# marcin-ochman/modular-slam

Measured on AMD Instinct MI355X. Metric: ORB keypoints extracted+matched /sec, 640×480 RGB-D, 1/2/4/8 GPU; HBM GB/s vs roofline, higher is better.
Workload: dtype u8

## Files before the change

modular-slam_amd/csrc/api.hip:

```cpp
#include "context.hpp"

#include <cfloat>
#include <climits>
#include <cmath>
#include <cstdio>
#include <cstring>
#include <cstdlib>
#include <algorithm>

using namespace mslam;

static thread_local std::string g_create_error;

#define ENTER(c)                                                                                                       \
    do                                                                                                                 \
    {                                                                                                                  \
        if(!(c))                                                                                                       \
            return MSLAM_HIP_E_INVALID;                                                                                \
        MSLAM_CHK(c, hipSetDevice((c)->p.device));                                                                     \
    } while(0)

static inline int cv_round_f(float v) { return (int)lrintf(v); }
static inline int cv_floor_f(float v)
{
    int i = (int)v;
    return i - (i > v);
}
static inline uint32_t sat_coef(float v)
{
    int iv = cv_round_f(v);
    iv = iv < SHRT_MIN ? SHRT_MIN : iv > SHRT_MAX ? SHRT_MAX : iv;
    return (uint32_t)(iv & 0xFFFF);
}

static void resize_table(int ssize, int dsize, bool clamp, std::vector<int32_t>& ofs, std::vector<uint32_t>& coef)
{
    const double inv_scale = (double)dsize / ssize;
    const double scale = 1. / inv_scale;
    for(int d = 0; d < dsize; ++d)
    {
        float f = (float)((d + 0.5) * scale - 0.5);
        int s = cv_floor_f(f);
        f -= s;
        if(clamp)
        {
            if(s < 0)
                f = 0, s = 0;
            if(s >= ssize - 1)
                f = 0, s = ssize - 1;
        }
        ofs.push_back(s);
        coef.push_back(sat_coef((1.f - f) * 2048) | (sat_coef(f * 2048) << 16));
    }
}

static void gaussian_taps_fixed(int taps[7])
{
    const int n = 7, n2 = 3;
    const double sigma = 2.0, scale2x = -0.125 / (sigma * sigma);
    double values[3], sum = 0;
    for(int i = 0, x = 1 - n; i < n2; ++i, x += 2)
    {
        values[i] = std::exp((double)(x * x) * scale2x);
        sum += values[i];
    }
    sum = sum * 2 + 1;
    const double mul1 = 1.0 / sum;
    double err = 0;
    long total = 0;
    for(int i = 0; i < n2; ++i)
    {
        const double adj = values[i] * mul1 * 256.0 + err;
        const long v0 = lrint(adj);
        err = adj - (double)v0;
        taps[i] = taps[n - 1 - i] = (int)v0;
        total += 2 * v0;
    }
    taps[n2] = (int)(256 - total);
}

static bool umax_table(int* out16)
{
    static const int expect[16] = {15, 15, 15, 15, 14, 14, 14, 13, 13, 12, 11, 10, 9, 8, 6, 3};
    int u[17] = {0};
    const int hp = 15;
    const unsigned vmax = (unsigned)std::floor(hp * std::sqrt(2.0) / 2 + 1);
    const unsigned vmin = (unsigned)std::ceil(hp * std::sqrt(2.0) / 2);
    for(unsigned v = 0; v <= vmax; ++v)
        u[v] = (int)std::round(std::sqrt((double)(hp * hp) - (double)(v * v)));
    for(unsigned v = hp, v0 = 0; vmin <= v; --v)
    {
        while(u[v0] == u[v0 + 1])
            ++v0;
        u[v] = (int)v0;
        ++v0;
    }
    std::memcpy(out16, u, sizeof(expect));
    return std::memcmp(u, expect, sizeof(expect)) == 0;
}

static void build_orient_weights(const int* umax, uint32_t* w )
{
    std::memset(w, 0, 2 * 256 * sizeof(uint32_t));
    for(int t = 0; t < 31 * 8; ++t)
    {
        const int v = t / 8 - 15, c = t % 8;
        for(int j = 0; j < 4; ++j)
        {
            const int u = -15 + 4 * c + j;
            const int au = u < 0 ? -u : u, av = v < 0 ? -v : v;
            if(au <= 15 && au <= umax[av])
            {
                w[t] |= (uint32_t)(uint8_t)(int8_t)u << (8 * j);
                w[256 + t] |= (uint32_t)(uint8_t)(int8_t)v << (8 * j);
            }
        }
    }
}

static int build_geometry(mslam_hip_ctx* c)
{
    const mslam_hip_params& p = c->p;
    Geometry& g = c->geom;
    g.n_levels = p.n_levels;
    g.W = p.width;
    g.H = p.height;
    g.blur_tiled = 0;
    float scale[kMaxLevels];
    scale[0] = 1.0f;
    for(int l = 1; l < p.n_levels; ++l)
        scale[l] = p.scale_factor * scale[l - 1];
    unsigned offset = 0;
    c->cells.clear();
    for(int l = 0; l < p.n_levels; ++l)
    {
        LevelGeom& lv = g.lv[l];
        const double s = scale[l];
        lv.w = l == 0 ? p.width : (int)std::round(p.width * 1.0 / s);
        lv.h = l == 0 ? p.height : (int)std::round(p.height * 1.0 / s);
        lv.scale = scale[l];
        if(lv.w <= 2 * kBorder + kOverlap || lv.h <= 2 * kBorder + kOverlap)
            return fail(c, MSLAM_HIP_E_INVALID,
                        "pyramid level " + std::to_string(l) + " is smaller than the 19-px border + one cell");
        if(lv.w > 4095 + kBorder || lv.h > 4095 + kBorder)
            return fail(c, MSLAM_HIP_E_INVALID, "frames larger than 4096 px per side are not supported");
        lv.pitch = (lv.w + kTileW - 1) & ~(kTileW - 1);
        lv.offset = (int)offset;
        offset += ((unsigned)lv.pitch * ((lv.h + kTileH - 1) & ~(kTileH - 1)) + 255u) & ~255u;
        lv.bw = lv.w - 2 * kBorder;
        lv.bh = lv.h - 2 * kBorder;

        const unsigned min_b = kBorder, max_bx = lv.w - kBorder, max_by = lv.h - kBorder;
        const unsigned num_cols = (max_bx - min_b) / kCell + 1, num_rows = (max_by - min_b) / kCell + 1;
        lv.cell_base = (int)c->cells.size();
        for(unsigned i = 0; i < num_rows; ++i)
        {
            const unsigned min_y = min_b + i * kCell;
            if(max_by - kOverlap <= min_y)
                continue;
            unsigned max_y = min_y + kCell + kOverlap;
            if(max_by < max_y)
                max_y = max_by;
            for(unsigned j = 0; j < num_cols; ++j)
            {
                const unsigned min_x = min_b + j * kCell;
                if(max_bx - kOverlap <= min_x)
                    continue;
                unsigned max_x = min_x + kCell + kOverlap;
                if(max_bx < max_x)
                    max_x = max_bx;
                CellDesc cd{};
                cd.level = (int16_t)l;
                cd.cw = (int16_t)(max_x - min_x);
                cd.ch = (int16_t)(max_y - min_y);
                cd.x0 = (int16_t)min_x;
                cd.y0 = (int16_t)min_y;
                cd.ox = (int16_t)(j * kCell);
                cd.oy = (int16_t)(i * kCell);
                c->cells.push_back(cd);
            }
        }
        lv.n_cells = (int)c->cells.size() - lv.cell_base;
        if(lv.n_cells > 2048)
            return fail(c, MSLAM_HIP_E_INVALID, "more than 2048 FAST cells on one level");

        lv.bsx = (lv.w + 3) / 4;

        const int min_x = kBorder, max_x = lv.w - kBorder, min_y = kBorder, max_y = lv.h - kBorder;
        const double ratio = (double)(max_x - min_x) / (max_y - min_y);
        if(ratio > 1)
        {
            lv.nxg = (int)std::round(ratio);
            lv.nyg = 1;
            lv.delta_x = (double)(max_x - min_x) / lv.nxg;
            lv.delta_y = max_y - min_y;
        }
        else
        {
            lv.nxg = 1;
            lv.nyg = (int)std::round(1 / ratio);
            lv.delta_x = max_x - min_y;
            lv.delta_y = (double)(max_y - min_y) / lv.nyg;
        }
        if(lv.nxg * lv.nyg > 64)
            return fail(c, MSLAM_HIP_E_INVALID, "aspect ratio beyond 64:1 is not supported");
    }
    g.slab = offset + 256;
    g.n_cells = (int)c->cells.size();
    return MSLAM_HIP_OK;
}

static int build_geometry_cv(mslam_hip_ctx* c)
{
    const mslam_hip_params& p = c->p;
    Geometry& g = c->geom;
    g.n_levels = p.n_levels;
    g.W = p.width;
    g.H = p.height;
    g.blur_tiled = 0;
    const double sf = (double)p.scale_factor;
    unsigned offset = 0;
    c->cells.clear();
    for(int l = 0; l < p.n_levels; ++l)
    {
        LevelGeom& lv = g.lv[l];
        lv = LevelGeom{};
        lv.scale = (float)std::pow(sf, (double)l);
        const float inv = 1.0f / lv.scale;
        lv.w = cv_round_f((float)p.width * inv);
        lv.h = cv_round_f((float)p.height * inv);
        if(lv.w < 16 || lv.h < 16)
            return fail(c, MSLAM_HIP_E_INVALID, "pyramid level " + std::to_string(l) + " is smaller than 16 px");
        if(lv.w > 4095 || lv.h > 4095)
            return fail(c, MSLAM_HIP_E_INVALID, "frames larger than 4095 px per side are not supported");
        lv.pitch = (lv.w + kTileW - 1) & ~(kTileW - 1);
        lv.offset = (int)offset;
        offset += ((unsigned)lv.pitch * ((lv.h + kTileH - 1) & ~(kTileH - 1)) + 255u) & ~255u;
        lv.bw = lv.w - 2 * kBorder;
        lv.bh = lv.h - 2 * kBorder;
        lv.bsx = (lv.w + 3) / 4;
    }
    g.slab = offset + 256;
    g.n_cells = 0;
    const float factor = (float)(1.0 / sf);
    float desired = (float)p.n_features * (1 - factor) / (1 - (float)std::pow((double)factor, (double)p.n_levels));
    int sum = 0;
    for(int l = 0; l < p.n_levels - 1; ++l)
    {
        c->cv_quota[l] = cv_round_f(desired);
        sum += c->cv_quota[l];
        desired *= factor;
    }
    c->cv_quota[p.n_levels - 1] = std::max(p.n_features - sum, 0);
    return MSLAM_HIP_OK;
}

static void exact_axis(int ssize, int dsize, std::vector<int32_t>& ofs, std::vector<uint32_t>& coef, int& dmin, int& dmax)
{
    const double scale = 1.0 / ((double)dsize / (double)ssize);
    dmin = 0;
    dmax = dsize;
    for(int d = 0; d < dsize; ++d)
    {
        const double fval = scale * ((double)d + 0.5) - 0.5;
        const int ival = (int)std::floor(fval);
        int o = 0;
        uint32_t c0 = 256, c1 = 0;
        if(ival >= 0 && ssize > 1)
        {
            if(ival < ssize - 1)
            {
                o = ival;
                c1 = (uint32_t)lrint((fval - (double)ival) * 256.0);
                c0 = 256 - c1;
            }
            else
            {
                o = ssize - 2;
                c0 = 0, c1 = 256;
                dmax = std::min(dmax, d);
            }
        }
        else
            dmin = std::max(dmin, d + 1);
        ofs.push_back(o);
        coef.push_back(c0 | (c1 << 16));
    }
}

extern "C" {

void mslam_hip_default_params(mslam_hip_params* p)
{
    std::memset(p, 0, sizeof(*p));
    p->width = 640;
    p->height = 480;
    p->max_batch = 1;
    p->n_levels = 8;
    p->scale_factor = 1.2f;
    p->ini_fast_thr = 20;
    p->min_fast_thr = 7;
    p->min_node_area = 1000;
    p->max_keypoints = 8192;
    p->max_candidates = 16384;
    p->device = 0;
    p->stream = nullptr;
    p->detector = MSLAM_HIP_DETECTOR_DISTRIBUTED;
    p->n_features = 1000;
    p->edge_threshold = 31;
}

int mslam_hip_abi_version(void) { return MSLAM_HIP_ABI_VERSION; }

const char* mslam_hip_last_error(const mslam_hip_ctx* ctx) { return ctx ? ctx->err.c_str() : g_create_error.c_str(); }

void mslam_hip_destroy(mslam_hip_ctx* c)
{
    if(!c)
        return;
    if(c->stream)
        (void)hipStreamSynchronize(c->stream);
    if(c->match_graph)
        (void)hipGraphExecDestroy(c->match_graph);
    for(auto& e : c->detect_graph)
        if(e)
            (void)hipGraphExecDestroy(e);
    if(c->stream_m)
        (void)hipStreamSynchronize(c->stream_m);
    for(auto& o : c->out)
    {
        if(o.ev_detect)
            (void)hipEventDestroy(o.ev_detect);
        if(o.ev_match)
            (void)hipEventDestroy(o.ev_match);
    }
    if(c->stream_m)
        (void)hipStreamDestroy(c->stream_m);
    for(auto& t : c->timers)
    {
        (void)hipEventDestroy(t.start);
        (void)hipEventDestroy(t.stop);
    }
    for(int k = 0; k < 4; ++k)
    {
        if(c->blur_stream[k])
        {
            (void)hipStreamSynchronize(c->blur_stream[k]);
            (void)hipStreamDestroy(c->blur_stream[k]);
        }
        if(c->ev_blur_fork[k])
            (void)hipEventDestroy(c->ev_blur_fork[k]);
        if(c->ev_blur_join[k])
            (void)hipEventDestroy(c->ev_blur_join[k]);
    }
    if(c->ev_fork)
        (void)hipEventDestroy(c->ev_fork);
    for(int k = 0; k < 4; ++k)
    {
        if(c->ev_join[k])
            (void)hipEventDestroy(c->ev_join[k]);
        if(c->side[k])
        {
            (void)hipStreamSynchronize(c->side[k]);
            (void)hipStreamDestroy(c->side[k]);
        }
    }
    if(c->bow)
        bow_destroy(c->bow);
    if(c->reloc)
        reloc_destroy(c->reloc);
    if(c->own_stream && c->stream)
        (void)hipStreamDestroy(c->stream);
    delete c;
}

static void build_quad_table(const std::vector<int32_t>& ofs, const std::vector<uint32_t>& coef, size_t x0, int dw,
                             int max_batch, std::vector<uint4>& qt, size_t& start_out, int& need_out)
{
    const int nq = (dw + 3) / 4;
    const size_t start = qt.size() / 3;
    bool ok = true;
    int need = 0;
    for(int q = 0; q < nq && ok; ++q)
    {
        const int first = ofs[x0 + 4 * q];
        const uint32_t base = (uint32_t)first & ~3u;
        uint32_t sel[4], cf[4], flags = 0;
        for(int k = 0; k < 4; ++k)
        {
            const int dx = std::min(4 * q + k, dw - 1);
            const int shift = ofs[x0 + dx] - (int)base;
            const uint32_t a0 = coef[x0 + dx] & 0xFFFF, a1 = coef[x0 + dx] >> 16;
            if(shift < 0 || shift > 10 || a0 > 0xFFF || a1 > 0xFFF)
                ok = false;
            const int upper = shift > 6 ? 1 : 0;
            flags |= (uint32_t)upper << k;
            sel[k] = 0x0c010c00u + (uint32_t)(shift - 4 * upper) * 0x00010001u;
            cf[k] = a0 | (a1 << 16);
        }
        need |= (int)flags;
        qt.push_back(make_uint4(base, flags, sel[0], sel[1]));
        qt.push_back(make_uint4(sel[2], sel[3], cf[0], cf[1]));
        qt.push_back(make_uint4(cf[2], cf[3], 0, 0));
    }
    if(!ok || (size_t)max_batch * nq >= (1u << 22))
    {
        qt.resize(start * 3);
        start_out = SIZE_MAX;
        return;
    }
    start_out = start;
    need_out = need;
}

static int create_impl(mslam_hip_ctx* c)
{
    const mslam_hip_params& p = c->p;
    const bool has_detector = !(p.width == 0 && p.height == 0);
    if((has_detector && (p.width <= 0 || p.height <= 0)) || p.max_batch < 1 || p.n_levels < 1 || p.n_levels > kMaxLevels ||
       !(p.scale_factor > 1.0f) || p.ini_fast_thr < 0 || p.ini_fast_thr > 255 || p.min_fast_thr < 0 ||
       p.min_fast_thr > p.ini_fast_thr || p.max_keypoints < 1 || p.max_keypoints > 65535 || p.max_candidates < 1 ||
       p.max_candidates > (1 << 22))
        return fail(c, MSLAM_HIP_E_INVALID, "invalid parameters");
    const bool cv_mode = p.detector == MSLAM_HIP_DETECTOR_CV_ORB;
    if((p.detector != MSLAM_HIP_DETECTOR_DISTRIBUTED && !cv_mode) ||
       (cv_mode && (p.n_features < 0 || p.edge_threshold < 19 || p.edge_threshold > 1024)))
        return fail(c, MSLAM_HIP_E_INVALID, "invalid detector parameters (cv::ORB mode needs edge_threshold >= 19: "
                                            "the descriptor pattern reaches 19 px)");
    int umax[16];
    if(!umax_table(umax))
        return fail(c, MSLAM_HIP_E_INVALID, "u_max table self-check failed");
    int taps[7];
    gaussian_taps_fixed(taps);
    static const int expect_taps[7] = {18, 34, 48, 56, 48, 34, 18};
    if(std::memcmp(taps, expect_taps, sizeof(taps)) != 0)
        return fail(c, MSLAM_HIP_E_INVALID, "gaussian tap self-check failed");
    set_blur_taps(taps);

    int rc = !has_detector ? MSLAM_HIP_OK : cv_mode ? build_geometry_cv(c) : build_geometry(c);
    if(rc)
        return rc;
    const Geometry& g = c->geom;

    int n_dev = 0;
    if(hipGetDeviceCount(&n_dev) != hipSuccess || n_dev <= 0)
        return fail(c, MSLAM_HIP_E_RUNTIME, "no HIP device available (the product path has no CPU fallback)");
    MSLAM_CHK(c, hipSetDevice(p.device));
    if(p.stream)
        c->stream = (hipStream_t)p.stream;
    else
    {
        MSLAM_CHK(c, hipStreamCreateWithFlags(&c->stream, hipStreamNonBlocking));
        c->own_stream = true;
    }

    {
        if(const char* ge = getenv("MSLAM_HIP_GRAPH"))
            c->use_graph = atoi(ge) != 0;
        const char* e = getenv("MSLAM_HIP_STREAMS");
        c->n_side = e ? std::max(1, std::min(atoi(e), 4)) : 2;
        MSLAM_CHK(c, hipEventCreateWithFlags(&c->ev_fork, hipEventDisableTiming));
        for(int k = 0; k < c->n_side; ++k)
        {
            MSLAM_CHK(c, hipStreamCreateWithFlags(&c->side[k], hipStreamNonBlocking));
            MSLAM_CHK(c, hipEventCreateWithFlags(&c->ev_join[k], hipEventDisableTiming));
        }
        const char* fb = getenv("MSLAM_HIP_FORK_BLUR");
        c->fork_blur = fb && atoi(fb) != 0;
        for(int k = 0; k < 4 && c->fork_blur; ++k)
        {
            MSLAM_CHK(c, hipStreamCreateWithFlags(&c->blur_stream[k], hipStreamNonBlocking));
            MSLAM_CHK(c, hipEventCreateWithFlags(&c->ev_blur_fork[k], hipEventDisableTiming));
            MSLAM_CHK(c, hipEventCreateWithFlags(&c->ev_blur_join[k], hipEventDisableTiming));
        }
    }
    if(has_detector && cv_mode)
    {
        std::vector<int32_t> ofs;
        std::vector<uint32_t> coef;
        c->cv_x.assign(p.n_levels, 0);
        c->cv_y.assign(p.n_levels, 0);
        c->cv_range.assign(p.n_levels, std::array<int, 4>{0, 0, 0, 0});
        c->cv_window12.assign(p.n_levels, 0);
        for(int l = 1; l < p.n_levels; ++l)
        {
            c->cv_x[l] = ofs.size();
            exact_axis(g.lv[l - 1].w, g.lv[l].w, ofs, coef, c->cv_range[l][0], c->cv_range[l][1]);
            c->cv_y[l] = ofs.size();
            exact_axis(g.lv[l - 1].h, g.lv[l].h, ofs, coef, c->cv_range[l][2], c->cv_range[l][3]);
            bool ok = true;
            const int dw = g.lv[l].w;
            for(int q = 0; q * 4 < dw && ok; ++q)
            {
                const int base = ofs[c->cv_x[l] + 4 * q] & ~3;
                for(int k = 0; k < 4; ++k)
                {
                    const int o = ofs[c->cv_x[l] + std::min(4 * q + k, dw - 1)];
                    ok = ok && o >= base && o + 1 - base <= 11;
                }
                ok = ok && base + 12 <= g.lv[l - 1].pitch;
            }
            c->cv_window12[l] = ok ? 1 : 0;
        }
        {
            std::vector<uint4> qt;
            c->rs_q.assign(p.n_levels, SIZE_MAX);
            c->rs_need.assign(p.n_levels, 0);
            for(int l = 1; l < p.n_levels; ++l)
                build_quad_table(ofs, coef, c->cv_x[l], g.lv[l].w, p.max_batch, qt, c->rs_q[l], c->rs_need[l]);
            qt.push_back(make_uint4(0, 0, 0, 0));
            MSLAM_CHK(c, c->d_rs_qt.alloc(qt.size()));
            MSLAM_CHK(c, hipMemcpy(c->d_rs_qt, qt.data(), qt.size() * 16, hipMemcpyHostToDevice));
        }
        ofs.push_back(0);
        coef.push_back(0);
        MSLAM_CHK(c, c->d_cv_ofs.alloc(ofs.size()));
        MSLAM_CHK(c, c->d_cv_coef.alloc(coef.size()));
        MSLAM_CHK(c, hipMemcpy(c->d_cv_ofs, ofs.data(), ofs.size() * 4, hipMemcpyHostToDevice));
        MSLAM_CHK(c, hipMemcpy(c->d_cv_coef, coef.data(), coef.size() * 4, hipMemcpyHostToDevice));
    }
    if(has_detector && !cv_mode)
    {
    MSLAM_CHK(c, c->d_cells.alloc(c->cells.size()));
    MSLAM_CHK(c, hipMemcpy(c->d_cells, c->cells.data(), c->cells.size() * sizeof(CellDesc), hipMemcpyHostToDevice));
    {
        std::vector<int32_t> ofs;
        std::vector<uint32_t> coef;
        c->rs_x.assign(p.n_levels, 0);
        c->rs_y.assign(p.n_levels, 0);
        for(int l = 1; l < p.n_levels; ++l)
        {
            c->rs_x[l] = ofs.size();
            resize_table(g.lv[l - 1].w, g.lv[l].w, true, ofs, coef);
            c->rs_y[l] = ofs.size();
            resize_table(g.lv[l - 1].h, g.lv[l].h, false, ofs, coef);
        }
        std::vector<uint4> qt;
        c->rs_q.assign(p.n_levels, SIZE_MAX);
        c->rs_need.assign(p.n_levels, 0);
        for(int l = 1; l < p.n_levels; ++l)
            build_quad_table(ofs, coef, c->rs_x[l], g.lv[l].w, p.max_batch, qt, c->rs_q[l], c->rs_need[l]);
        qt.push_back(make_uint4(0, 0, 0, 0));
        MSLAM_CHK(c, c->d_rs_qt.alloc(qt.size()));
        MSLAM_CHK(c, hipMemcpy(c->d_rs_qt, qt.data(), qt.size() * 16, hipMemcpyHostToDevice));
        ofs.push_back(0);
        coef.push_back(0);
        MSLAM_CHK(c, c->d_rs_ofs.alloc(ofs.size()));
        MSLAM_CHK(c, c->d_rs_coef.alloc(coef.size()));
        MSLAM_CHK(c, hipMemcpy(c->d_rs_ofs, ofs.data(), ofs.size() * 4, hipMemcpyHostToDevice));
        MSLAM_CHK(c, hipMemcpy(c->d_rs_coef, coef.data(), coef.size() * 4, hipMemcpyHostToDevice));
    }
    }
    MSLAM_CHK(c, c->d_ratio_thr.alloc(257));
    {
        uint32_t w[2 * 256];
        build_orient_weights(umax, w);
        MSLAM_CHK(c, c->d_orient_w.alloc(2 * 256));
        MSLAM_CHK(c, hipMemcpy(c->d_orient_w, w, sizeof(w), hipMemcpyHostToDevice));
    }

    const size_t B = (size_t)p.max_batch, L = (size_t)p.n_levels, cap = (size_t)p.max_candidates;
    const size_t K = (size_t)p.max_keypoints;
    MSLAM_CHK(c, c->h_out.alloc(16 + K * 52));
    MSLAM_CHK(c, c->d_flags.alloc(1));
    MSLAM_CHK(c, hipMemset(c->d_flags, 0, 4));
    if(has_detector)
    {
    {
        uint32_t ok = 0;
        launch_denorm_selfcheck(c->d_flags, c->stream);
        MSLAM_CHK(c, hipGetLastError());
        MSLAM_CHK(c, hipMemcpyAsync(&ok, c->d_flags, 4, hipMemcpyDeviceToHost, c->stream));
        MSLAM_CHK(c, hipStreamSynchronize(c->stream));
        MSLAM_CHK(c, hipMemset(c->d_flags, 0, 4));
        if(ok != 1u)
            return fail(c, MSLAM_HIP_E_RUNTIME, "v_pk_minimum3_f16 / v_pk_maximum3_f16 do not preserve f16 denormals in this build "
                                                "(the FAST score kernels need .amdhsa_float_denorm_mode_16_64 3): refusing to run");
    }
    MSLAM_CHK(c, c->d_stage.alloc((size_t)p.width * p.height * 3));
    MSLAM_CHK(c, c->d_pyr.alloc(B * g.slab + 256));
    MSLAM_CHK(c, c->d_blur.alloc(B * g.slab + 256));
    {
        {
            const char* e = getenv("MSLAM_HIP_FUSED_LEVELS");
            const int want = e ? atoi(e) : kMaxLevels;
            const char* k = getenv("MSLAM_HIP_LEVEL_K6");
            const char* ks = getenv("MSLAM_HIP_LEVEL_K6_SMALL");
            c->level_k6_small = ks ? std::max(0, atoi(ks)) : 0;
            {
                const char* lc = getenv("MSLAM_HIP_LEVEL_CHAIN");
                const char* lf = getenv("MSLAM_HIP_LEVEL_CHAIN_FRAMES");
                const char* lw = getenv("MSLAM_HIP_LEVEL_CHAIN_WAVES");
                const char* lk = getenv("MSLAM_HIP_LEVEL_CHAIN_K6");
                c->level_chain = lc ? atoi(lc) : 0;
                c->level_chain_frames = lf ? std::max(1, std::min(64, atoi(lf))) : 2;
                c->level_chain_waves = lw ? atoi(lw) : 8;
                if(c->level_chain_waves != 4)
                    c->level_chain_waves = 8;
                c->level_chain_k6 = lk ? std::max(1, std::min(9, atoi(lk))) : 9;
            }
            c->level_k6 = k ? std::max(1, atoi(k)) : 9;
            const bool fits = (p.width & 3) == 0 && (double)B * p.width * p.height * 3 < 4294967296.0 &&
                              (double)B * g.slab < 4294901760.0  && (size_t)B * (p.width / 4) < (1u << 22) && p.height >= 8;
            int n_fused = fits ? 1 : 0;
            while(n_fused >= 1 && n_fused < p.n_levels && c->rs_q[n_fused] != SIZE_MAX && g.lv[n_fused].h >= 8 &&
                  (size_t)B * ((g.lv[n_fused].w + 3) / 4) < (1u << 22))
                ++n_fused;
            c->fused_levels = std::max(0, std::min(want, n_fused));
            const char* t = getenv("MSLAM_HIP_TILED_BLUR");
            c->geom.blur_tiled = c->fused_levels == p.n_levels && !(t && atoi(t) == 0) ? 1 : 0;
        }
        std::vector<BlurWave> bw;
        build_blur_waves(g, c->fused_levels, bw);
        c->blur_wpf = (int)bw.size();
        if(!bw.empty())
        {
            MSLAM_CHK(c, c->d_blur_waves.alloc(bw.size()));
            MSLAM_CHK(c, hipMemcpy(c->d_blur_waves, bw.data(), bw.size() * sizeof(BlurWave), hipMemcpyHostToDevice));
        }
    }
    MSLAM_CHK(c, c->d_cell_cnt.alloc(B * g.n_cells));
    MSLAM_CHK(c, c->d_cell_kp.alloc(B * g.n_cells * (size_t)kCellCap));
    QuadArgs& q = c->quad;
    MSLAM_CHK(c, c->q_cand.alloc(B * L * cap));
    MSLAM_CHK(c, c->q_cand_cnt.alloc(B * L));
    MSLAM_CHK(c, c->q_sel.alloc(B * L * cap));
    MSLAM_CHK(c, c->q_sel_cnt.alloc(B * L));
    MSLAM_CHK(c, c->q_kp_node.alloc(B * L * cap));
    MSLAM_CHK(c, c->q_nodes_a.alloc(B * L * cap));
    MSLAM_CHK(c, c->q_nodes_b.alloc(B * L * cap));
    MSLAM_CHK(c, c->q_ncnt_a.alloc(B * L * cap));
    MSLAM_CHK(c, c->q_ncnt_b.alloc(B * L * cap));
    MSLAM_CHK(c, c->q_child_cnt.alloc(B * L * cap * 4));
    MSLAM_CHK(c, c->q_ninfo.alloc(B * L * cap));
    MSLAM_CHK(c, c->q_best.alloc(B * L * cap));
    q.cand = c->q_cand, q.cand_cnt = c->q_cand_cnt, q.sel = c->q_sel, q.sel_cnt = c->q_sel_cnt, q.kp_node = c->q_kp_node;
    q.nodes_a = c->q_nodes_a, q.nodes_b = c->q_nodes_b, q.ncnt_a = c->q_ncnt_a, q.ncnt_b = c->q_ncnt_b;
    q.child_cnt = c->q_child_cnt, q.ninfo = c->q_ninfo, q.best = c->q_best;
    q.cell_cnt = c->d_cell_cnt;
    q.cell_kp = c->d_cell_kp;
    q.flags = c->d_flags;
    q.cand_cap = p.max_candidates;
    q.min_size = p.min_node_area;
    }

    for(auto& o : c->out)
    {
        MSLAM_CHK(c, o.xy.alloc((B + 1) * K * 2));
        MSLAM_CHK(c, o.desc.alloc((B + 1) * K * 32));
        MSLAM_CHK(c, o.octave.alloc((B + 1) * K));
        MSLAM_CHK(c, o.angle.alloc((B + 1) * K));
        MSLAM_CHK(c, o.response.alloc((B + 1) * K));
        MSLAM_CHK(c, o.count.alloc(B + 1));
        MSLAM_CHK(c, hipMemset(o.count, 0, (B + 1) * 4));
        MSLAM_CHK(c, o.idx0.alloc(B * K));
        MSLAM_CHK(c, o.idx1.alloc(B * K));
        MSLAM_CHK(c, o.dist0.alloc(B * K));
        MSLAM_CHK(c, o.dist1.alloc(B * K));
        MSLAM_CHK(c, o.mfrom.alloc(B * K));
        MSLAM_CHK(c, o.mto.alloc(B * K));
        MSLAM_CHK(c, o.mcount.alloc(B));
        MSLAM_CHK(c, hipMemset(o.mcount, 0, B * 4));
        MSLAM_CHK(c, hipEventCreateWithFlags(&o.ev_detect, hipEventDisableTiming));
        MSLAM_CHK(c, hipEventCreateWithFlags(&o.ev_match, hipEventDisableTiming));
    }
    MSLAM_CHK(c, hipStreamCreateWithFlags(&c->stream_m, hipStreamNonBlocking));
    {
        const char* e = getenv("MSLAM_HIP_OVERLAP_MATCH");
        c->overlap_match = !(e && atoi(e) == 0);
        auto on = [](const char* name) { const char* v = getenv(name); return !v || atoi(v) != 0; };
        c->knob_mirror_results = on("MSLAM_HIP_MIRROR_RESULTS");
        c->knob_zero_copy = on("MSLAM_HIP_ZERO_COPY_FRAME");
        c->knob_match_graph = on("MSLAM_HIP_MATCH_GRAPH");
        const char* zm = getenv("MSLAM_HIP_ZERO_COPY_MAX_BYTES");
        c->zero_copy_max_bytes = zm ? (size_t)atoll(zm) : (size_t)1200000;
        const char* m = getenv("MSLAM_HIP_MATCHER");
        c->matcher_kind = (m && std::strcmp(m, "popcount") == 0) ? MSLAM_HIP_MATCHER_POPCOUNT : MSLAM_HIP_MATCHER_AUTO;
    }
    c->cur = 0;
    MSLAM_CHK(c, hipDeviceSynchronize());
    return MSLAM_HIP_OK;
}

int mslam_hip_create(const mslam_hip_params* p, mslam_hip_ctx** out)
{
    if(!p || !out)
    {
        g_create_error = "null argument";
        return MSLAM_HIP_E_INVALID;
    }
    *out = nullptr;
    mslam_hip_ctx* c = new mslam_hip_ctx();
    c->p = *p;
    const int rc = create_impl(c);
    if(rc != MSLAM_HIP_OK)
    {
        g_create_error = c->err;
        mslam_hip_destroy(c);
        return rc;
    }
    *out = c;
    return MSLAM_HIP_OK;
}

constexpr int kMinChunk = 8;

static int check_flags(mslam_hip_ctx* c)
{
    uint32_t f = 0;
    MSLAM_CHK(c, hipStreamSynchronize(c->stream_m));
    MSLAM_CHK(c, hipMemcpyAsync(&f, c->d_flags, 4, hipMemcpyDeviceToHost, c->stream));
    MSLAM_CHK(c, hipStreamSynchronize(c->stream));
    if(f == 0)
        return MSLAM_HIP_OK;
    MSLAM_CHK(c, hipMemsetAsync(c->d_flags, 0, 4, c->stream));
    std::string m = "capacity exceeded:";
    if(f & kFlagCandOverflow)
        m += " FAST candidates on a level > max_candidates;";
    if(f & kFlagKpOverflow)
        m += " keypoints in a frame > max_keypoints;";
    if(f & kFlagQuadNoConverge)
        m += " quadtree pass limit;";
    if(f & kFlagDbFull)
        m += " the BoW database is full (mslam_hip_bow_db_reserve);";
    if(f & kFlagBowPackOverflow)
        m += " a BoW vector has more words than the exchange format's k_max;";
    if(f & kFlagPackOverflow)
        m += " packed batch results larger than the buffer given to mslam_hip_pack_batch_dev (header.bytes);";
    if(f & kFlagUnionOverflow)
        m += " a union of store entries has more distinct landmarks than max_keypoints (mslam_hip_kf_union_dev);";
    return fail(c, MSLAM_HIP_E_CAPACITY, m);
}

int mslam_hip_sync(mslam_hip_ctx* c)
{
    ENTER(c);
    return check_flags(c);
}

__global__ __launch_bounds__(256) void k_pack_results(const float* __restrict__ xy, const uint8_t* __restrict__ desc,
                                                      const int32_t* __restrict__ octave, const float* __restrict__ angle,
                                                      const float* __restrict__ response, const int32_t* __restrict__ count,
                                                      const uint32_t* __restrict__ flags, uint8_t* __restrict__ h, int K)
{
    const int n = min(max(*count, 0), K);
    const int tid = blockIdx.x * 256 + threadIdx.x, nt = gridDim.x * 256;
    if(tid == 0)
    {
        reinterpret_cast<int32_t*>(h)[0] = *count;
        reinterpret_cast<uint32_t*>(h)[1] = *flags;
    }
    uint2* h_xy = reinterpret_cast<uint2*>(h + 16);
    uint2* h_desc = reinterpret_cast<uint2*>(h + 16 + (size_t)K * 8);
    uint32_t* h_oct = reinterpret_cast<uint32_t*>(h + 16 + (size_t)K * 40);
    uint32_t* h_ang = h_oct + K;
    uint32_t* h_resp = h_ang + K;
    for(int i = tid; i < 4 * n; i += nt)
        h_desc[i] = reinterpret_cast<const uint2*>(desc)[i];
    for(int i = tid; i < n; i += nt)
    {
        h_xy[i] = reinterpret_cast<const uint2*>(xy)[i];
        h_oct[i] = reinterpret_cast<const uint32_t*>(octave)[i];
        h_ang[i] = reinterpret_cast<const uint32_t*>(angle)[i];
        h_resp[i] = reinterpret_cast<const uint32_t*>(response)[i];
    }
}

__global__ __launch_bounds__(256) void k_carry_prev(uint4* __restrict__ dst, const uint4* __restrict__ src, int32_t* __restrict__ dst_count,
                                                    const int32_t* __restrict__ src_count, int K)
{
    const int n = min(max(*src_count, 0), K);
    const int tid = blockIdx.x * 256 + threadIdx.x;
    if(tid == 0)
        *dst_count = *src_count;
    for(int i = tid; i < 2 * n; i += gridDim.x * 256)
        dst[i] = src[i];
}

static void enqueue_resize_blur(mslam_hip_ctx* c, int l, const int32_t* yofs, const uint32_t* ycoef, int exact, int f0, int nf,
                                int k6, hipStream_t cs, ResizeBlurArgs* chain_out = nullptr)
{
    const Geometry& g = c->geom;
    const LevelGeom &sl = g.lv[l - 1], &dl = g.lv[l];
    ResizeBlurArgs ra{};
    ra.pyr = c->d_pyr;
    ra.blur = c->d_blur;
    ra.slab = g.slab;
    ra.src_off = sl.offset, ra.sh = sl.h, ra.spitch = sl.pitch;
    ra.dst_off = dl.offset, ra.dw = dl.w, ra.dh = dl.h, ra.dpitch = dl.pitch;
    ra.qt = c->d_rs_qt + 3 * c->rs_q[l];
    ra.yofs = yofs;
    ra.ycoef = ycoef;
    ra.frame0 = f0, ra.n_frames = nf;
    ra.quads = (dl.w + 3) / 4;
    ra.inv_quads = 1.0f / (float)ra.quads;
    if(k6 == 0 && dl.h >= 380)
        k6 = 1;
    ra.k6 = std::max(k6 == 0 ? 0 : 1, std::min(std::min(k6, 9), (dl.h - 2) / 6));
    {
        const long waves_x = ((long)nf * ra.quads + 61) / 62;
        while(ra.k6 > 2 && waves_x * ((dl.h + 6 * ra.k6 + 1) / (6 * ra.k6 + 2)) < 2048)
            --ra.k6;
    }
    ra.need_mask = c->rs_need[l];
    ra.exact = exact;
    ra.blur_tiled = g.blur_tiled;
    ra.always_load = nf < 8 ? 1 : 0;
    ra.bk = make_blur_k();
    if(chain_out)
    {
        *chain_out = ra;
        return;
    }
    launch_resize_blur(ra, cs);
}

static int enqueue_detect(mslam_hip_ctx* c, const uint8_t* d_bgr, int n_frames)
{
    const Geometry& g = c->geom;
    const size_t K = (size_t)c->p.max_keypoints;
    hipStream_t s = c->stream;
    const int k6_batch = n_frames >= 8 ? c->level_k6 : c->level_k6_small;
    const int n_chunks = (c->profiling || n_frames < 2 * kMinChunk) ? 1 : std::min<int>(c->n_side, n_frames / kMinChunk);
    if(n_chunks > 1)
        MSLAM_CHK(c, hipEventRecord(c->ev_fork, s));
    for(int k = 0; k < n_chunks; ++k)
    {
        const int f0 = (int)((long long)n_frames * k / n_chunks), f1 = (int)((long long)n_frames * (k + 1) / n_chunks);
        const int nf = f1 - f0;
        hipStream_t cs = n_chunks > 1 ? c->side[k] : s;
        if(n_chunks > 1)
            MSLAM_CHK(c, hipStreamWaitEvent(cs, c->ev_fork, 0));
        const bool cv_mode = c->p.detector == MSLAM_HIP_DETECTOR_CV_ORB;
        bool chained = false;
        if(c->level_chain && !cv_mode && nf >= 8 && c->fused_levels == g.n_levels && g.n_levels <= kChainLevels && g.blur_tiled)
        {
            StageScope t(c, "levels", cs);
            GrayBlurArgs ga{};
            ga.bgr = d_bgr;
            ga.pyr = c->d_pyr;
            ga.blur = c->d_blur;
            ga.W = g.W, ga.H = g.H, ga.pitch = g.lv[0].pitch;
            ga.slab = g.slab;
            ga.n_frames = nf, ga.frame0 = f0;
            ga.quads = g.W / 4;
            ga.inv_quads = 1.0f / (float)ga.quads;
            ga.k6 = 1;
            ga.blur_tiled = g.blur_tiled;
            ga.bk = make_blur_k();
            ResizeBlurArgs lv[kChainLevels - 1];
            for(int l = 1; l < g.n_levels; ++l)
                enqueue_resize_blur(c, l, c->d_rs_ofs + c->rs_y[l], c->d_rs_coef + c->rs_y[l], 0, f0, nf, k6_batch, cs, &lv[l - 1]);
            chained = launch_level_chain(ga, lv, g.n_levels - 1, c->level_chain_frames, c->level_chain_waves, c->level_chain_k6, cs);
        }
        if(!chained)
        {
            StageScope t(c, "gray", cs);
            if(c->fused_levels >= 1)
            {
                GrayBlurArgs ga{};
                ga.bgr = d_bgr;
                ga.pyr = c->d_pyr;
                ga.blur = c->d_blur;
                ga.W = g.W, ga.H = g.H, ga.pitch = g.lv[0].pitch;
                ga.slab = g.slab;
                ga.n_frames = nf, ga.frame0 = f0;
                ga.quads = g.W / 4;
                ga.inv_quads = 1.0f / (float)ga.quads;
                ga.k6 = std::max(k6_batch == 0 && g.H < 380 ? 0 : 1, std::min(k6_batch, (g.H - 2) / 6));
                ga.blur_tiled = g.blur_tiled;
                ga.bk = make_blur_k();
                launch_gray_blur(ga, cs);
            }
            else
                launch_gray(d_bgr, c->d_pyr, g, f0, nf, cs);
        }
        if(cv_mode)
        {
            {
                StageScope t(c, "resize", cs);
                for(int l = 1; l < g.n_levels; ++l)
                {
                    const LevelGeom &sl = g.lv[l - 1], &dl = g.lv[l];
                    if(l < c->fused_levels)
                    {
                        enqueue_resize_blur(c, l, c->d_cv_ofs + c->cv_y[l], c->d_cv_coef + c->cv_y[l], 1, f0, nf, k6_batch, cs);
                        continue;
                    }
                    if(c->rs_q[l] != SIZE_MAX)
                    {
                        ResizeColArgs ca{};
                        ca.pyr = c->d_pyr;
                        ca.slab = g.slab;
                        ca.src_off = sl.offset, ca.sh = sl.h, ca.spitch = sl.pitch;
                        ca.dst_off = dl.offset, ca.dw = dl.w, ca.dh = dl.h, ca.dpitch = dl.pitch;
                        ca.qt = c->d_rs_qt + 3 * c->rs_q[l];
                        ca.yofs = c->d_cv_ofs + c->cv_y[l];
                        ca.ycoef = c->d_cv_coef + c->cv_y[l];
                        ca.frame0 = f0, ca.n_frames = nf;
                        ca.quads = (dl.w + 3) / 4;
                        ca.inv_quads = 1.0f / (float)ca.quads;
                        ca.R = 8;
                        ca.need_mask = c->rs_need[l];
                        ca.exact = 1;
                        launch_resize_col(ca, cs);
                        continue;
                    }
                    ExactResizeArgs ra{};
                    ra.pyr = c->d_pyr;
                    ra.slab = g.slab;
                    ra.src_off = sl.offset, ra.sw = sl.w, ra.sh = sl.h, ra.spitch = sl.pitch;
                    ra.dst_off = dl.offset, ra.dw = dl.w, ra.dh = dl.h, ra.dpitch = dl.pitch;
                    ra.xofs = c->d_cv_ofs + c->cv_x[l];
                    ra.xcoef = c->d_cv_coef + c->cv_x[l];
                    ra.yofs = c->d_cv_ofs + c->cv_y[l];
                    ra.ycoef = c->d_cv_coef + c->cv_y[l];
                    ra.xmin = c->cv_range[l][0], ra.xmax = c->cv_range[l][1];
                    ra.ymin = c->cv_range[l][2], ra.ymax = c->cv_range[l][3];
                    ra.window12 = c->cv_window12[l];
                    ra.frame0 = f0;
                    launch_resize_exact(ra, nf, cs);
                }
            }
            CvSelectArgs sa{};
            sa.cand = c->quad.cand, sa.cand_cnt = c->quad.cand_cnt;
            sa.tmp_kp = c->quad.kp_node, sa.tmp_resp = reinterpret_cast<float*>(c->quad.ninfo);
            sa.sel = c->quad.sel, sa.sel_resp = reinterpret_cast<float*>(c->quad.best), sa.sel_cnt = c->quad.sel_cnt;
            sa.flags = c->d_flags;
            sa.cand_cap = c->p.max_candidates;
            sa.edge = c->p.edge_threshold;
            sa.std_order = c->cv_order == MSLAM_HIP_CV_ORDER_LIBSTDCXX ? 1 : 0;
            for(int l = 0; l < g.n_levels; ++l)
                sa.quota[l] = c->cv_quota[l];
            {
                StageScope t(c, "fast", cs);
                launch_zero_u32(c->quad.cand_cnt + (size_t)f0 * g.n_levels, nf * g.n_levels, cs);
                launch_fast_tiles(c->d_pyr, g, c->p.ini_fast_thr, sa, f0, nf, cs);
            }
            {
                StageScope t(c, "select", cs);
                launch_cv_select(c->d_pyr, g, sa, f0, nf, cs);
            }
        }
        else
        {
        if(!chained)
        {
            StageScope t(c, "resize", cs);
            for(int l = 1; l < g.n_levels; ++l)
            {
                if(l < c->fused_levels)
                {
                    enqueue_resize_blur(c, l, c->d_rs_ofs + c->rs_y[l], c->d_rs_coef + c->rs_y[l], 0, f0, nf, k6_batch, cs);
                    continue;
                }
                if(c->rs_q[l] != SIZE_MAX)
                {
                    const LevelGeom &sl = g.lv[l - 1], &dl = g.lv[l];
                    ResizeColArgs ra{};
                    ra.pyr = c->d_pyr;
                    ra.slab = g.slab;
                    ra.src_off = sl.offset;
                    ra.sh = sl.h;
                    ra.spitch = sl.pitch;
                    ra.dst_off = dl.offset;
                    ra.dw = dl.w;
                    ra.dh = dl.h;
                    ra.dpitch = dl.pitch;
                    ra.qt = c->d_rs_qt + 3 * c->rs_q[l];
                    ra.yofs = c->d_rs_ofs + c->rs_y[l];
                    ra.ycoef = c->d_rs_coef + c->rs_y[l];
                    ra.frame0 = f0;
                    ra.n_frames = nf;
                    ra.quads = (dl.w + 3) / 4;
                    ra.inv_quads = 1.0f / (float)ra.quads;
                    ra.R = 8;
                    ra.need_mask = c->rs_need[l];
                    launch_resize_col(ra, cs);
                }
                else
                    launch_resize(c->d_pyr, g, l, c->d_rs_ofs + c->rs_x[l], c->d_rs_coef + c->rs_x[l],
                                  c->d_rs_ofs + c->rs_y[l], c->d_rs_coef + c->rs_y[l], f0, nf, cs);
            }
        }
        {
            StageScope t(c, "fast", cs);
            launch_fast(c->d_pyr, g, c->d_cells, c->d_cell_cnt, c->d_cell_kp, c->p.ini_fast_thr, c->p.min_fast_thr, f0,
                        nf, cs);
        }
        const bool blur_needed = c->fused_levels < g.n_levels;
        const bool forked = c->fork_blur && !c->profiling && blur_needed;
        if(forked)
        {
            MSLAM_CHK(c, hipEventRecord(c->ev_blur_fork[k], cs));
            MSLAM_CHK(c, hipStreamWaitEvent(c->blur_stream[k], c->ev_blur_fork[k], 0));
            {
                StageScope t(c, "blur", c->blur_stream[k]);
                launch_blur(c->d_pyr, c->d_blur, g, c->d_blur_waves, c->blur_wpf, f0, nf, c->blur_stream[k]);
            }
            MSLAM_CHK(c, hipEventRecord(c->ev_blur_join[k], c->blur_stream[k]));
        }
        {
            StageScope t(c, "quadtree", cs);
            launch_quadtree(g, c->quad, f0, nf, cs);
        }
        if(forked)
            MSLAM_CHK(c, hipStreamWaitEvent(cs, c->ev_blur_join[k], 0));
        else if(blur_needed)
        {
            StageScope t(c, "blur", cs);
            launch_blur(c->d_pyr, c->d_blur, g, c->d_blur_waves, c->blur_wpf, f0, nf, cs);
        }
        }
        if(cv_mode && c->fused_levels < g.n_levels)
        {
            StageScope t(c, "blur", cs);
            launch_blur(c->d_pyr, c->d_blur, g, c->d_blur_waves, c->blur_wpf, f0, nf, cs);
        }
        {
            StageScope t(c, "describe", cs);
            DescArgs a{};
            a.pyr = c->d_pyr;
            a.blur = c->d_blur;
            a.sel = c->quad.sel;
            a.sel_cnt = c->quad.sel_cnt;
            a.orient_w = c->d_orient_w;
            a.cand_cap = c->p.max_candidates;
            a.max_kp = c->p.max_keypoints;
            a.xy = cur_out(c).xy + K * 2;
            a.desc = cur_out(c).desc + K * 32;
            a.octave = cur_out(c).octave + K;
            a.angle = cur_out(c).angle + K;
            a.response = cur_out(c).response + K;
            a.count = cur_out(c).count + 1;
            a.flags = c->d_flags;
            if(cv_mode)
            {
                a.sel_resp = reinterpret_cast<const float*>(c->quad.best);
                a.cv_mode = 1;
            }
            if(c->mirror_results && n_frames == 1)
                a.h_mirror = c->h_out.dev();
            launch_describe(g, a, f0, nf, cs);
        }
        if(n_chunks > 1)
        {
            MSLAM_CHK(c, hipEventRecord(c->ev_join[k], cs));
            MSLAM_CHK(c, hipStreamWaitEvent(s, c->ev_join[k], 0));
        }
    }
    MSLAM_CHK(c, hipGetLastError());
    return MSLAM_HIP_OK;
}

static int detect_prologue(mslam_hip_ctx* c)
{
    const size_t K = (size_t)c->p.max_keypoints;
    hipStream_t s = c->stream;
    if(!c->inplace_timing)
        c->timers_used = 0;
    if(c->n_last > 0)
    {
        const int prev = c->cur, nxt = prev ^ 1;
        if(c->out[nxt].match_pending)
        {
            MSLAM_CHK(c, hipStreamWaitEvent(s, c->out[nxt].ev_match, 0));
            c->out[nxt].match_pending = false;
        }
        const size_t last = (size_t)c->n_last;
        hipLaunchKernelGGL(k_carry_prev, dim3(16), dim3(256), 0, s, reinterpret_cast<uint4*>(c->out[nxt].desc.get()),
                           reinterpret_cast<const uint4*>(c->out[prev].desc + last * K * 32), c->out[nxt].count,
                           c->out[prev].count + last, (int)K);
        MSLAM_CHK(c, hipGetLastError());
        c->have_prev = true;
        c->cur = nxt;
    }
    return MSLAM_HIP_OK;
}

int mslam_hip_detect_batch_dev(mslam_hip_ctx* c, const uint8_t* d_bgr, int n_frames)
{
    ENTER(c);
    if(c->p.width == 0)
        return fail(c, MSLAM_HIP_E_INVALID, "detect_batch_dev: this context was created without a detector (0 x 0)");
    if(!d_bgr || n_frames < 1 || n_frames > c->p.max_batch)
        return fail(c, MSLAM_HIP_E_INVALID, "detect_batch_dev: n_frames outside [1, max_batch]");
    int rc = detect_prologue(c);
    if(rc)
        return rc;
    rc = enqueue_detect(c, d_bgr, n_frames);
    if(rc)
        return rc;
    MSLAM_CHK(c, hipEventRecord(c->out[c->cur].ev_detect, c->stream));
    c->n_last = n_frames;
    ++c->detect_seq;
    return MSLAM_HIP_OK;
}

int mslam_hip_get_batch_view(mslam_hip_ctx* c, mslam_hip_batch_view* v)
{
    if(!c || !v)
        return MSLAM_HIP_E_INVALID;
    const size_t K = (size_t)c->p.max_keypoints;
    v->n_frames = c->n_last;
    v->capacity = c->p.max_keypoints;
    v->xy = cur_out(c).xy + K * 2;
    v->desc = cur_out(c).desc + K * 32;
    v->octave = cur_out(c).octave + K;
    v->angle = cur_out(c).angle + K;
    v->response = cur_out(c).response + K;
    v->count = cur_out(c).count + 1;
    v->match_from = cur_out(c).mfrom;
    v->match_to = cur_out(c).mto;
    v->match_count = cur_out(c).mcount;
    return MSLAM_HIP_OK;
}

int mslam_hip_detect(mslam_hip_ctx* c, const uint8_t* bgr, int width, int height, int max_out, float* xy,
                     uint8_t* desc, int32_t* octave, float* angle, float* response, int* n_out)
{
    ENTER(c);
    if(n_out)
        *n_out = 0;
    if(!bgr || !n_out || max_out < 0 || (max_out > 0 && (!xy || !desc)))
        return fail(c, MSLAM_HIP_E_INVALID, "detect: null argument");
    if(c->p.width == 0)
        return fail(c, MSLAM_HIP_E_INVALID, "detect: this context was created without a detector (0 x 0)");
    if(width != c->p.width || height != c->p.height)
        return fail(c, MSLAM_HIP_E_INVALID, "detect: frame size differs from the context's");
    const size_t K = (size_t)c->p.max_keypoints;
    uint8_t* h = c->h_out;
    uint8_t* h_xy = h + 16;
    uint8_t* h_desc = h_xy + K * 8;
    uint8_t* h_oct = h_desc + K * 32;
    uint8_t* h_ang = h_oct + K * 4;
    uint8_t* h_resp = h_ang + K * 4;
    const bool mirror_env = c->knob_mirror_results;
    struct MirrorScope
    {
        mslam_hip_ctx* c;
        MirrorScope(mslam_hip_ctx* cc, bool on) : c(cc) { c->mirror_results = on; }
        ~MirrorScope() { c->mirror_results = false; }
    } mirror_scope(c, mirror_env);
    auto enqueue_results = [&]() -> int {
        if(c->mirror_results)
            return MSLAM_HIP_OK;
        const mslam_out_set& o = cur_out(c);
        hipLaunchKernelGGL(k_pack_results, dim3(32), dim3(256), 0, c->stream, o.xy + K * 2, o.desc + K * 32, o.octave + K,
                           o.angle + K, o.response + K, o.count + 1, c->d_flags, c->h_out.dev(), (int)K);
        MSLAM_CHK(c, hipGetLastError());
        return MSLAM_HIP_OK;
    };
    MSLAM_CHK(c, hipStreamSynchronize(c->stream_m));
    int rc = detect_prologue(c);
    if(rc)
        return rc;
    const bool zero_copy = c->knob_zero_copy && (size_t)width * height * 3 <= c->zero_copy_max_bytes;
    const uint8_t* frame_src = c->d_stage;
    if(zero_copy)
    {
        if(!c->h_stage)
        {
            MSLAM_CHK(c, c->h_stage.alloc((size_t)width * height * 3));
        }
        std::memcpy(c->h_stage, bgr, (size_t)width * height * 3);
        frame_src = c->h_stage.dev();
    }
    else
        MSLAM_CHK(c, hipMemcpyAsync(c->d_stage, bgr, (size_t)width * height * 3, hipMemcpyHostToDevice, c->stream));
    if(!c->profiling && !c->inplace_timing && c->use_graph)
    {
        hipGraphExec_t& exec = c->detect_graph[c->cur];
        if(!exec)
        {
            hipGraph_t graph = nullptr;
            MSLAM_CHK(c, hipStreamBeginCapture(c->stream, hipStreamCaptureModeRelaxed));
            rc = enqueue_detect(c, frame_src, 1);
            if(!rc)
                rc = enqueue_results();
            const hipError_t e = hipStreamEndCapture(c->stream, &graph);
            const hipError_t e_inst = (!rc && e == hipSuccess) ? hipGraphInstantiate(&exec, graph, nullptr, nullptr, 0) : hipSuccess;
            if(graph)
                (void)hipGraphDestroy(graph);
            if(e_inst != hipSuccess)
                exec = nullptr;
            if(rc)
                return rc;
            MSLAM_CHK(c, e);
            MSLAM_CHK(c, e_inst);
        }
        MSLAM_CHK(c, hipGraphLaunch(exec, c->stream));
    }
    else
    {
        rc = enqueue_detect(c, frame_src, 1);
        if(rc)
            return rc;
        rc = enqueue_results();
        if(rc)
            return rc;
    }
    MSLAM_CHK(c, hipEventRecord(c->out[c->cur].ev_detect, c->stream));
    c->n_last = 1;
    ++c->detect_seq;
    MSLAM_CHK(c, hipStreamSynchronize(c->stream));
    uint32_t flags;
    int32_t n;
    std::memcpy(&n, h, 4);
    std::memcpy(&flags, h + 4, 4);
    if(flags)
        return check_flags(c);
    *n_out = n;
    if(n > max_out)
        return fail(c, MSLAM_HIP_E_CAPACITY, "detect: max_out smaller than the number of keypoints");
    if(n == 0)
        return MSLAM_HIP_OK;
    std::memcpy(xy, h_xy, (size_t)n * 8);
    std::memcpy(desc, h_desc, (size_t)n * 32);
    if(octave)
        std::memcpy(octave, h_oct, (size_t)n * 4);
    if(angle)
        std::memcpy(angle, h_ang, (size_t)n * 4);
    if(response)
        std::memcpy(response, h_resp, (size_t)n * 4);
    return MSLAM_HIP_OK;
}

static int upload_ratio_table(mslam_hip_ctx* c, double ratio)
{
    if(ratio == c->ratio_cached)
        return MSLAM_HIP_OK;
    int32_t thr[257];
    for(int d1 = 0; d1 <= 256; ++d1)
    {
        int n = 0;
        for(int d0 = 0; d0 <= 256; ++d0)
            if((double)(float)d0 < ratio * (double)(float)d1)
                ++n;
            else
                break;
        thr[d1] = n;
    }
    MSLAM_CHK(c, hipStreamSynchronize(c->stream_m));
    MSLAM_CHK(c, hipMemcpyAsync(c->d_ratio_thr, thr, sizeof(thr), hipMemcpyHostToDevice, c->stream));
    MSLAM_CHK(c, hipStreamSynchronize(c->stream));
    c->ratio_cached = ratio;
    return MSLAM_HIP_OK;
}
__attribute__((visibility("hidden"))) int mslam_ratio_table(mslam_hip_ctx* c, double ratio) { return upload_ratio_table(c, ratio); }

int mslam_hip_match_batch_dev(mslam_hip_ctx* c, double ratio, int chain_previous)
{
    ENTER(c);
    if(c->n_last < 1)
        return fail(c, MSLAM_HIP_E_INVALID, "match_batch_dev: no detect batch to match");
    int rc = upload_ratio_table(c, ratio);
    if(rc)
        return rc;
    const size_t K = (size_t)c->p.max_keypoints;
    const int first = (chain_previous && c->have_prev) ? 0 : 1;
    const int n_pairs = c->n_last - first;
    c->match_seq = c->detect_seq;
    const bool own = c->overlap_match && !c->profiling;
    hipStream_t s = own ? c->stream_m : c->stream;
    if(own)
        MSLAM_CHK(c, hipStreamWaitEvent(s, c->out[c->cur].ev_detect, 0));
    if(first == 1)
        MSLAM_CHK(c, hipMemsetAsync(cur_out(c).mcount, 0, 4, s));
    if(n_pairs > 0)
    {
        MatchArgs m{};
        m.from_desc = cur_out(c).desc + (size_t)(first + 1) * K * 32;
        m.to_desc = cur_out(c).desc + (size_t)first * K * 32;
        m.from_stride = m.to_stride = (long long)K * 32;
        m.from_cnt = cur_out(c).count + first + 1;
        m.to_cnt = cur_out(c).count + first;
        m.cap = c->p.max_keypoints;
        m.cap_from = c->p.max_keypoints;
        m.popcount_only = c->matcher_kind == MSLAM_HIP_MATCHER_POPCOUNT;
        m.idx0 = cur_out(c).idx0 + (size_t)first * K;
        m.idx1 = cur_out(c).idx1 + (size_t)first * K;
        m.dist0 = cur_out(c).dist0 + (size_t)first * K;
        m.dist1 = cur_out(c).dist1 + (size_t)first * K;
        {
            StageScope t(c, "match_knn2", s);
            c->last_match_kernel = launch_match_knn2(m, n_pairs, s);
        }
        RatioArgs r{};
        r.idx0 = m.idx0;
        r.dist0 = m.dist0;
        r.dist1 = m.dist1;
        r.from_cnt = m.from_cnt;
        r.to_cnt = m.to_cnt;
        r.cap = m.cap;
        r.thr = c->d_ratio_thr;
        r.from_idx = cur_out(c).mfrom + (size_t)first * K;
        r.to_idx = cur_out(c).mto + (size_t)first * K;
        r.n_out = cur_out(c).mcount + first;
        {
            StageScope t(c, "ratio_compact", s);
            launch_ratio_compact(r, n_pairs, s);
        }
    }
    MSLAM_CHK(c, hipGetLastError());
    if(own)
    {
        MSLAM_CHK(c, hipEventRecord(c->out[c->cur].ev_match, s));
        c->out[c->cur].match_pending = true;
    }
    return MSLAM_HIP_OK;
}

constexpr int kHostMatchSlices = 8;
static int host_match_prepare(mslam_hip_ctx* c, const uint8_t* from_desc, int n_from, const uint8_t* to_desc, int n_to)
{
    if(n_from > c->hm_from_cap || n_to > c->hm_to_cap)
    {
        MSLAM_CHK(c, hipStreamSynchronize(c->stream));
        const int from_cap = std::max(n_from, std::max(c->hm_from_cap, 2048)), to_cap = std::max(n_to, std::max(c->hm_to_cap, 2048));
        c->hm_from_cap = c->hm_to_cap = 0;
        c->d_hm_to = nullptr;
        if(c->match_graph)
        {
            (void)hipGraphExecDestroy(c->match_graph);
            c->match_graph = nullptr;
        }
        MSLAM_CHK(c, c->d_hm_from.alloc((size_t)(from_cap + to_cap) * 32 + 16));
        MSLAM_CHK(c, c->d_hm_out.alloc((size_t)to_cap * 6 + 4));
        MSLAM_CHK(c, c->d_hm_partial.alloc((size_t)kHostMatchSlices * 2 * to_cap));
        MSLAM_CHK(c, c->h_hm.alloc((size_t)(from_cap + to_cap) * 32 + 16 + ((size_t)to_cap * 2 + 4) * 4));
        c->hm_from_cap = from_cap;
        c->hm_to_cap = to_cap;
    }
    c->d_hm_to = c->d_hm_from + (size_t)n_from * 32;
    if(n_from > 0)
        std::memcpy(c->h_hm, from_desc, (size_t)n_from * 32);
    std::memcpy(c->h_hm + (size_t)n_from * 32, to_desc, (size_t)n_to * 32);
    MSLAM_CHK(c, hipMemcpyAsync(c->d_hm_from, c->h_hm, (size_t)(n_from + n_to) * 32, hipMemcpyHostToDevice, c->stream));
    return MSLAM_HIP_OK;
}

static void host_match_args(mslam_hip_ctx* c, int n_from, int n_to, MatchArgs& m)
{
    const size_t cap = (size_t)c->hm_to_cap;
    m = MatchArgs{};
    m.from_desc = c->d_hm_from;
    m.to_desc = c->d_hm_to;
    m.n_from_fixed = n_from;
    m.n_to_fixed = n_to;
    m.cap = n_to;
    m.idx0 = c->d_hm_out;
    m.idx1 = c->d_hm_out + cap;
    m.dist0 = c->d_hm_out + 2 * cap;
    m.dist1 = c->d_hm_out + 3 * cap;
    m.popcount_only = c->matcher_kind == MSLAM_HIP_MATCHER_POPCOUNT;
    m.partial = c->d_hm_partial;
    m.n_slices = std::max(1, std::min(kHostMatchSlices, (n_from + 255) / 256));
}

static int host_match_graph(mslam_hip_ctx* c, const uint8_t* from_desc, int n_from, const uint8_t* to_desc, int n_to, int* n_out,
                            int32_t* from_idx, int32_t* to_idx)
{
    const size_t fcap = (size_t)c->hm_from_cap, tcap = (size_t)c->hm_to_cap;
    uint8_t* h_cnt = c->h_hm + (fcap + tcap) * 32;
    if(n_from > 0)
        std::memcpy(c->h_hm, from_desc, (size_t)n_from * 32);
    if(n_to > 0)
        std::memcpy(c->h_hm + fcap * 32, to_desc, (size_t)n_to * 32);
    const int32_t counts[4] = {n_from, n_to, 0, 0};
    std::memcpy(h_cnt, counts, sizeof(counts));
    int32_t* res_dev = reinterpret_cast<int32_t*>(c->h_hm.dev() + (fcap + tcap) * 32 + 16);
    const int32_t* res = reinterpret_cast<const int32_t*>(c->h_hm + (fcap + tcap) * 32 + 16);
    if(!c->match_graph || c->match_graph_from_cap != c->hm_from_cap || c->match_graph_to_cap != c->hm_to_cap ||
       c->match_graph_kind != c->matcher_kind)
    {
        if(c->match_graph)
            (void)hipGraphExecDestroy(c->match_graph);
        c->match_graph = nullptr;
        hipGraph_t graph = nullptr;
        MSLAM_CHK(c, hipStreamBeginCapture(c->stream, hipStreamCaptureModeRelaxed));
        hipError_t e = hipMemcpyAsync(c->d_hm_from, c->h_hm, (fcap + tcap) * 32 + 16, hipMemcpyHostToDevice, c->stream);
        const int32_t* d_cnt = reinterpret_cast<const int32_t*>(c->d_hm_from + (fcap + tcap) * 32);
        MatchArgs m{};
        m.from_desc = c->d_hm_from;
        m.to_desc = c->d_hm_from + fcap * 32;
        m.from_cnt = d_cnt;
        m.to_cnt = d_cnt + 1;
        m.cap = (int)tcap;
        m.cap_from = (int)fcap;
        m.idx0 = c->d_hm_out;
        m.idx1 = c->d_hm_out + tcap;
        m.dist0 = c->d_hm_out + 2 * tcap;
        m.dist1 = c->d_hm_out + 3 * tcap;
        m.popcount_only = c->matcher_kind == MSLAM_HIP_MATCHER_POPCOUNT;
        m.partial = c->d_hm_partial;
        m.n_slices = kHostMatchSlices;
        RatioArgs r{};
        r.idx0 = m.idx0;
        r.dist0 = m.dist0;
        r.dist1 = m.dist1;
        r.from_cnt = m.from_cnt;
        r.to_cnt = m.to_cnt;
        r.cap = (int)tcap;
        r.thr = c->d_ratio_thr;
        r.from_idx = res_dev;
        r.to_idx = res_dev + tcap;
        r.n_out = res_dev + 2 * tcap;
        if(launch_match_ratio_single(m, r, c->stream))
            c->last_match_kernel = 1;
        else
        {
            c->last_match_kernel = launch_match_knn2(m, 1, c->stream);
            launch_ratio_compact(r, 1, c->stream);
        }
        const hipError_t e_launch = hipGetLastError();
        const hipError_t e2 = hipStreamEndCapture(c->stream, &graph);
        hipError_t e3 = (e == hipSuccess && e_launch == hipSuccess && e2 == hipSuccess)
                            ? hipGraphInstantiate(&c->match_graph, graph, nullptr, nullptr, 0)
                            : hipSuccess;
        if(graph)
            (void)hipGraphDestroy(graph);
        if(e3 != hipSuccess)
            c->match_graph = nullptr;
        MSLAM_CHK(c, e);
        MSLAM_CHK(c, e_launch);
        MSLAM_CHK(c, e2);
        MSLAM_CHK(c, e3);
        c->match_graph_from_cap = c->hm_from_cap;
        c->match_graph_to_cap = c->hm_to_cap;
        c->match_graph_kind = c->matcher_kind;
        c->match_graph_kernel = c->last_match_kernel;
    }
    c->last_match_kernel = c->match_graph_kernel;
    MSLAM_CHK(c, hipGraphLaunch(c->match_graph, c->stream));
    MSLAM_CHK(c, hipStreamSynchronize(c->stream));
    const int32_t n = res[2 * tcap];
    if(n < 0 || n > n_to || (size_t)n > tcap)
        return fail(c, MSLAM_HIP_E_RUNTIME, "match: the kernel reported an impossible match count");
    std::memcpy(from_idx, res, (size_t)n * 4);
    std::memcpy(to_idx, res + tcap, (size_t)n * 4);
    *n_out = n;
    return MSLAM_HIP_OK;
}

int mslam_hip_join_matcher(mslam_hip_ctx* c)
{
    ENTER(c);
    for(auto& o : c->out)
        if(o.match_pending)
            MSLAM_CHK(c, hipStreamWaitEvent(c->stream, o.ev_match, 0));
    return MSLAM_HIP_OK;
}

int mslam_hip_set_matcher(mslam_hip_ctx* c, int kind)
{
    if(!c)
        return MSLAM_HIP_E_INVALID;
    if(kind != MSLAM_HIP_MATCHER_AUTO && kind != MSLAM_HIP_MATCHER_POPCOUNT)
        return fail(c, MSLAM_HIP_E_INVALID, "set_matcher: unknown kind");
    c->matcher_kind = kind;
    return MSLAM_HIP_OK;
}

int mslam_hip_get_matcher(const mslam_hip_ctx* c) { return c ? c->matcher_kind : -1; }

int mslam_hip_set_cv_keypoint_order(mslam_hip_ctx* c, int order)
{
    ENTER(c);
    if(order != MSLAM_HIP_CV_ORDER_LIBSTDCXX && order != MSLAM_HIP_CV_ORDER_RASTER)
        return fail(c, MSLAM_HIP_E_INVALID, "set_cv_keypoint_order: unknown order");
    if(order == c->cv_order)
        return MSLAM_HIP_OK;
    MSLAM_CHK(c, hipStreamSynchronize(c->stream));
    for(auto& e : c->detect_graph)
        if(e)
        {
            (void)hipGraphExecDestroy(e);
            e = nullptr;
        }
    c->cv_order = order;
    return MSLAM_HIP_OK;
}
int mslam_hip_last_match_kernel(const mslam_hip_ctx* c) { return c ? c->last_match_kernel : -1; }

int mslam_hip_match_knn2(mslam_hip_ctx* c, const uint8_t* from_desc, int n_from, const uint8_t* to_desc, int n_to,
                         int32_t* idx0, int32_t* idx1, int32_t* dist0, int32_t* dist1)
{
    ENTER(c);
    if(n_from < 0 || n_to < 0 || (n_from > 0 && !from_desc) || (n_to > 0 && (!to_desc || !idx0 || !idx1 || !dist0 || !dist1)))
        return fail(c, MSLAM_HIP_E_INVALID, "match_knn2: bad argument");
    if(n_from > 65535)
        return fail(c, MSLAM_HIP_E_INVALID, "match_knn2: more than 65535 train descriptors are not supported");
    if(n_to == 0)
        return MSLAM_HIP_OK;
    int rc = host_match_prepare(c, from_desc, n_from, to_desc, n_to);
    if(rc)
        return rc;
    MatchArgs m;
    host_match_args(c, n_from, n_to, m);
    c->last_match_kernel = launch_match_knn2(m, 1, c->stream);
    MSLAM_CHK(c, hipGetLastError());
    MSLAM_CHK(c, hipMemcpyAsync(idx0, m.idx0, (size_t)n_to * 4, hipMemcpyDeviceToHost, c->stream));
    MSLAM_CHK(c, hipMemcpyAsync(idx1, m.idx1, (size_t)n_to * 4, hipMemcpyDeviceToHost, c->stream));
    MSLAM_CHK(c, hipMemcpyAsync(dist0, m.dist0, (size_t)n_to * 4, hipMemcpyDeviceToHost, c->stream));
    MSLAM_CHK(c, hipMemcpyAsync(dist1, m.dist1, (size_t)n_to * 4, hipMemcpyDeviceToHost, c->stream));
    MSLAM_CHK(c, hipStreamSynchronize(c->stream));
    return MSLAM_HIP_OK;
}

int mslam_hip_match(mslam_hip_ctx* c, const uint8_t* from_desc, int n_from, const uint8_t* to_desc, int n_to,
                    double ratio, int32_t* from_idx, int32_t* to_idx, int* n_out)
{
    ENTER(c);
    if(n_out)
        *n_out = 0;
    if(!n_out || n_from < 0 || n_to < 0 || (n_from > 0 && !from_desc) || (n_to > 0 && (!to_desc || !from_idx || !to_idx)))
        return fail(c, MSLAM_HIP_E_INVALID, "match: bad argument");
    if(n_from > 65535)
        return fail(c, MSLAM_HIP_E_INVALID, "match: more than 65535 train descriptors are not supported");
    if(n_to == 0 || n_from < 2)
        return MSLAM_HIP_OK;
    int rc = upload_ratio_table(c, ratio);
    if(rc)
        return rc;
    const bool graph_env = c->knob_match_graph;
    if(graph_env && c->use_graph && !c->profiling && !c->inplace_timing && c->hm_from_cap >= n_from && c->hm_to_cap >= n_to &&
       c->hm_from_cap + c->hm_to_cap <= 2 * (n_from + n_to) + 2048 && c->hm_from_cap <= 32736)
        return host_match_graph(c, from_desc, n_from, to_desc, n_to, n_out, from_idx, to_idx);
    rc = host_match_prepare(c, from_desc, n_from, to_desc, n_to);
    if(rc)
        return rc;
    if(graph_env && c->use_graph && !c->profiling && !c->inplace_timing && c->hm_from_cap <= 32736 &&
       c->hm_from_cap + c->hm_to_cap <= 2 * (n_from + n_to) + 2048)
    {
        MSLAM_CHK(c, hipStreamSynchronize(c->stream));
        return host_match_graph(c, from_desc, n_from, to_desc, n_to, n_out, from_idx, to_idx);
    }
    MatchArgs m;
    host_match_args(c, n_from, n_to, m);
    c->last_match_kernel = launch_match_knn2(m, 1, c->stream);
    const size_t cap = (size_t)c->hm_to_cap;
    RatioArgs r{};
    r.idx0 = m.idx0;
    r.dist0 = m.dist0;
    r.dist1 = m.dist1;
    r.n_from_fixed = n_from;
    r.n_to_fixed = n_to;
    r.cap = n_to;
    r.thr = c->d_ratio_thr;
    int32_t* res_dev = reinterpret_cast<int32_t*>(c->h_hm.dev() + (size_t)(c->hm_from_cap + c->hm_to_cap) * 32 + 16);
    const int32_t* res = reinterpret_cast<const int32_t*>(c->h_hm + (size_t)(c->hm_from_cap + c->hm_to_cap) * 32 + 16);
    r.from_idx = res_dev;
    r.to_idx = res_dev + cap;
    r.n_out = res_dev + 2 * cap;
    launch_ratio_compact(r, 1, c->stream);
    MSLAM_CHK(c, hipGetLastError());
    MSLAM_CHK(c, hipStreamSynchronize(c->stream));
    const int32_t n = res[2 * cap];
    std::memcpy(from_idx, res, (size_t)n * 4);
    std::memcpy(to_idx, res + cap, (size_t)n * 4);
    *n_out = n;
    return MSLAM_HIP_OK;
}

int mslam_hip_level_geometry(mslam_hip_ctx* c, int* widths, int* heights, float* scales)
{
    if(!c)
        return MSLAM_HIP_E_INVALID;
    for(int l = 0; l < c->geom.n_levels; ++l)
    {
        if(widths)
            widths[l] = c->geom.lv[l].w;
        if(heights)
            heights[l] = c->geom.lv[l].h;
        if(scales)
            scales[l] = c->geom.lv[l].scale;
    }
    return MSLAM_HIP_OK;
}

int mslam_hip_debug_read(mslam_hip_ctx* c, int what, int frame, int level, void* dst, size_t dst_bytes,
                         size_t* n_items)
{
    ENTER(c);
    if(c->p.width == 0 || frame < 0 || frame >= c->p.max_batch || level < 0 || level >= c->geom.n_levels || !dst || !n_items)
        return fail(c, MSLAM_HIP_E_INVALID, "debug_read: bad argument");
    MSLAM_CHK(c, hipStreamSynchronize(c->stream));
    const LevelGeom& lv = c->geom.lv[level];
    if(what == MSLAM_HIP_DBG_PYRAMID || what == MSLAM_HIP_DBG_BLURRED)
    {
        const size_t need = (size_t)lv.w * lv.h;
        *n_items = need;
        if(dst_bytes < need)
            return fail(c, MSLAM_HIP_E_CAPACITY, "debug_read: buffer too small");
        const uint8_t* src = (what == MSLAM_HIP_DBG_PYRAMID ? c->d_pyr : c->d_blur) + (size_t)frame * c->geom.slab + lv.offset;
        if(what == MSLAM_HIP_DBG_BLURRED && c->geom.blur_tiled)
        {
            std::vector<uint8_t> tmp((size_t)lv.pitch * ((lv.h + kTileH - 1) & ~(kTileH - 1)));
            MSLAM_CHK(c, hipMemcpy(tmp.data(), src, tmp.size(), hipMemcpyDeviceToHost));
            uint8_t* out = static_cast<uint8_t*>(dst);
            for(int y = 0; y < lv.h; ++y)
                for(int x = 0; x < lv.w; ++x)
                    out[(size_t)y * lv.w + x] = tmp[tiled_off((unsigned)lv.pitch, x, y)];
            return MSLAM_HIP_OK;
        }
        MSLAM_CHK(c, hipMemcpy2D(dst, lv.w, src, lv.pitch, lv.w, lv.h, hipMemcpyDeviceToHost));
        return MSLAM_HIP_OK;
    }
    if(what == MSLAM_HIP_DBG_CANDIDATES || what == MSLAM_HIP_DBG_SELECTED)
    {
        const size_t slot = (size_t)frame * c->geom.n_levels + level;
        const bool cand = what == MSLAM_HIP_DBG_CANDIDATES;
        uint32_t n = 0;
        MSLAM_CHK(c, hipMemcpy(&n, (cand ? c->quad.cand_cnt : c->quad.sel_cnt) + slot, 4, hipMemcpyDeviceToHost));
        n = std::min<uint32_t>(n, (uint32_t)c->p.max_candidates);
        *n_items = n;
        if(dst_bytes < (size_t)n * 12)
            return fail(c, MSLAM_HIP_E_CAPACITY, "debug_read: buffer too small");
        std::vector<uint32_t> tmp(n);
        if(n)
            MSLAM_CHK(c, hipMemcpy(tmp.data(), (cand ? c->quad.cand : c->quad.sel) + slot * (size_t)c->p.max_candidates,
                                   (size_t)n * 4, hipMemcpyDeviceToHost));
        if(cand && c->p.detector == MSLAM_HIP_DETECTOR_CV_ORB && c->cv_order == MSLAM_HIP_CV_ORDER_LIBSTDCXX && n > (uint32_t)kSelLds)
            std::sort(tmp.begin(), tmp.end());
        float* out = static_cast<float*>(dst);
        for(uint32_t i = 0; i < n; ++i)
        {
            out[3 * i] = (float)kp_x(tmp[i]);
            out[3 * i + 1] = (float)kp_y(tmp[i]);
            out[3 * i + 2] = (float)kp_score(tmp[i]);
        }
        if(c->p.detector == MSLAM_HIP_DETECTOR_CV_ORB && !cand)
        {
            std::vector<float> resp(n);
            if(n)
                MSLAM_CHK(c, hipMemcpy(resp.data(), reinterpret_cast<const float*>(c->quad.best) + slot * (size_t)c->p.max_candidates,
                                       (size_t)n * 4, hipMemcpyDeviceToHost));
            for(uint32_t i = 0; i < n; ++i)
            {
                out[3 * i] += (float)kBorder;
                out[3 * i + 1] += (float)kBorder;
                out[3 * i + 2] = resp[i];
            }
        }
        return MSLAM_HIP_OK;
    }
    if(what == MSLAM_HIP_DBG_CELLS && c->p.detector == MSLAM_HIP_DETECTOR_DISTRIBUTED)
    {
        *n_items = (size_t)lv.n_cells;
        if(dst_bytes < (size_t)lv.n_cells * 24)
            return fail(c, MSLAM_HIP_E_CAPACITY, "debug_read: buffer too small");
        int32_t* out = static_cast<int32_t*>(dst);
        for(int i = 0; i < lv.n_cells; ++i)
        {
            const CellDesc& cd = c->cells[(size_t)lv.cell_base + i];
            const int32_t rec[6] = {cd.x0, cd.y0, cd.cw, cd.ch, cd.ox, cd.oy};
            std::memcpy(out + 6 * i, rec, sizeof(rec));
        }
        return MSLAM_HIP_OK;
    }
    if(what == MSLAM_HIP_DBG_FORMS)
    {
        *n_items = 2;
        if(dst_bytes < 8)
            return fail(c, MSLAM_HIP_E_CAPACITY, "debug_read: buffer too small");
        const int32_t rec[2] = {c->fused_levels, c->geom.blur_tiled};
        std::memcpy(dst, rec, sizeof(rec));
        return MSLAM_HIP_OK;
    }
    return fail(c, MSLAM_HIP_E_INVALID, "debug_read: unknown item");
}

int mslam_hip_debug_counts(mslam_hip_ctx* c, int what, int32_t* out, int n_frames)
{
    ENTER(c);
    if(c->p.width == 0 || !out || n_frames < 1 || (what != MSLAM_HIP_DBG_CANDIDATES && what != MSLAM_HIP_DBG_SELECTED))
        return fail(c, MSLAM_HIP_E_INVALID, "debug_counts: bad argument");
    MSLAM_CHK(c, hipStreamSynchronize(c->stream));
    const int rows = std::min(n_frames, std::max(c->n_last, 1));
    MSLAM_CHK(c, hipMemcpy(out, what == MSLAM_HIP_DBG_CANDIDATES ? c->quad.cand_cnt : c->quad.sel_cnt,
                           (size_t)rows * c->geom.n_levels * 4, hipMemcpyDeviceToHost));
    return MSLAM_HIP_OK;
}

int mslam_hip_copy_to_host(mslam_hip_ctx* c, void* dst_host, const void* src_dev, size_t bytes)
{
    ENTER(c);
    if(!dst_host || !src_dev)
        return fail(c, MSLAM_HIP_E_INVALID, "copy_to_host: null pointer");
    MSLAM_CHK(c, hipStreamSynchronize(c->stream_m));
    MSLAM_CHK(c, hipStreamSynchronize(c->stream));
    MSLAM_CHK(c, hipMemcpy(dst_host, src_dev, bytes, hipMemcpyDeviceToHost));
    return MSLAM_HIP_OK;
}

int mslam_hip_set_profiling(mslam_hip_ctx* c, int enable)
{
    if(!c)
        return MSLAM_HIP_E_INVALID;
    c->profiling = enable == 1;
    c->inplace_timing = enable == 2;
    c->timers_used = 0;
    return MSLAM_HIP_OK;
}

int mslam_hip_get_stage_times(mslam_hip_ctx* c, const char** names, float* ms, int cap, int* n)
{
    ENTER(c);
    if(!n)
        return fail(c, MSLAM_HIP_E_INVALID, "get_stage_times: null output");
    MSLAM_CHK(c, hipStreamSynchronize(c->stream_m));
    MSLAM_CHK(c, hipStreamSynchronize(c->stream));
    int k = 0;
    for(size_t i = 0; i < c->timers_used && k < cap; ++i, ++k)
    {
        float t = 0;
        MSLAM_CHK(c, hipEventElapsedTime(&t, c->timers[i].start, c->timers[i].stop));
        if(names)
            names[k] = c->timers[i].name;
        if(ms)
            ms[k] = t;
    }
    *n = k;
    if(c->inplace_timing)
        c->timers_used = 0;
    return MSLAM_HIP_OK;
}

}
```

modular-slam_amd/csrc/common.hpp:

```cpp
#pragma once
#include <hip/hip_runtime.h>
#include <cstdint>
#include <cstddef>

namespace mslam
{

constexpr int kMaxLevels = 16;
constexpr int kBorder = 19;
constexpr int kCell = 64;
constexpr int kOverlap = 6;
constexpr int kCellCap = 1024;

constexpr size_t al256(size_t x) { return (x + 255) & ~(size_t)255; }

struct LevelGeom
{
    int w, h;
    int pitch;
    int offset;
    float scale;
    int bw, bh;
    int cell_base;
    int n_cells;
    int bsx;
    int nxg, nyg;
    double delta_x, delta_y;
};

struct Geometry
{
    int n_levels;
    int W, H;
    int n_cells;
    int frame0;
    unsigned slab;
    int blur_tiled;
    LevelGeom lv[kMaxLevels];
};

#ifndef MSLAM_TILE_W
#define MSLAM_TILE_W 64
#endif
constexpr int kTileW = MSLAM_TILE_W, kTileH = 128 / kTileW;
constexpr int kTileWLog = kTileW == 64 ? 6 : kTileW == 32 ? 5 : 4, kTileHLog = 7 - kTileWLog;
static_assert(kTileW == 16 || kTileW == 32 || kTileW == 64, "tile width");
__host__ __device__ __forceinline__ unsigned tiled_off(unsigned pitch, int x, int y)
{
    return (unsigned)(y >> kTileHLog) * (pitch * (unsigned)kTileH) + (unsigned)(x >> kTileWLog) * 128u +
           (unsigned)(y & (kTileH - 1)) * (unsigned)kTileW + (unsigned)(x & (kTileW - 1));
}
template <class P>
__device__ __forceinline__ P lds_ptr(uint32_t off)
{
#if defined(__HIP_DEVICE_COMPILE__)
    return (P)off;
#else
    return (P)(uintptr_t)off;
#endif
}
struct CellDesc
{
    int16_t level, cw, ch, pad;
    int16_t x0, y0;
    int16_t ox, oy;
};

constexpr int kBlurRows = 32;

__host__ __device__ inline uint32_t pack_kp(int x, int y, int score) { return ((uint32_t)y << 20) | ((uint32_t)x << 8) | (uint32_t)score; }
__host__ __device__ inline int kp_x(uint32_t p) { return (int)((p >> 8) & 0xFFFu); }
__host__ __device__ inline int kp_y(uint32_t p) { return (int)(p >> 20); }
__host__ __device__ inline int kp_score(uint32_t p) { return (int)(p & 0xFFu); }

enum : uint32_t
{
    kFlagCandOverflow = 1u,
    kFlagKpOverflow = 2u,
    kFlagQuadNoConverge = 4u,
    kFlagBowPackOverflow = 8u,
    kFlagDbFull = 16u,
    kFlagPackOverflow = 32u,
    kFlagUnionOverflow = 64u
};

void launch_gray(const uint8_t* d_bgr, uint8_t* d_pyr, const Geometry& g, int frame0, int n_frames, hipStream_t s);
void launch_resize(uint8_t* d_pyr, const Geometry& g, int level, const int32_t* d_xofs, const uint32_t* d_xcoef,
                   const int32_t* d_yofs, const uint32_t* d_ycoef, int frame0, int n_frames, hipStream_t s);
struct ResizeColArgs
{
    uint8_t* pyr;
    unsigned slab;
    int src_off, sh, spitch, dst_off, dw, dh, dpitch;
    const uint4* qt;
    const int32_t* yofs;
    const uint32_t* ycoef;
    int frame0, n_frames;
    int quads;
    float inv_quads;
    int R;
    int need_mask;
    int exact;
};
void launch_resize_col(const ResizeColArgs& a, hipStream_t s);
void launch_fast(const uint8_t* d_pyr, const Geometry& g, const CellDesc* d_cells, uint32_t* d_cell_cnt,
                 uint32_t* d_cell_kp, int ini_thr, int min_thr, int frame0, int n_frames, hipStream_t s);
void launch_denorm_selfcheck(uint32_t* d_out, hipStream_t s);
struct QuadArgs
{
    const uint32_t* cell_cnt;
    const uint32_t* cell_kp;
    uint32_t* cand;
    uint32_t* cand_cnt;
    uint32_t* sel;
    uint32_t* sel_cnt;
    uint32_t* kp_node;
    uint2* nodes_a;
    uint2* nodes_b;
    uint32_t* ncnt_a;
    uint32_t* ncnt_b;
    uint32_t* child_cnt;
    uint32_t* ninfo;
    uint32_t* best;
    uint32_t* flags;
    int cand_cap;
    unsigned min_size;
};
void launch_quadtree(const Geometry& g, const QuadArgs& a, int frame0, int n_frames, hipStream_t s);
struct BlurK
{
    uint32_t ta[3], tb[4], tc[4];
    uint32_t t01, t23, t45, t6;
};
BlurK make_blur_k();
struct GrayBlurArgs
{
    const uint8_t* bgr;
    uint8_t* pyr;
    uint8_t* blur;
    int W, H, pitch;
    unsigned slab;
    int n_frames, frame0;
    int quads;
    float inv_quads;
    int k6;
    int waves_per_xcd;
    int blur_tiled;
    BlurK bk;
};
void launch_gray_blur(const GrayBlurArgs& a, hipStream_t s);
struct ResizeBlurArgs
{
    uint8_t* pyr;
    uint8_t* blur;
    unsigned slab;
    int src_off, sh, spitch, dst_off, dw, dh, dpitch;
    const uint4* qt;
    const int32_t* yofs;
    const uint32_t* ycoef;
    int frame0, n_frames;
    int quads;
    float inv_quads;
    int k6;
    int need_mask;
    int exact;
    int waves_per_xcd;
    int blur_tiled;
    int always_load;
    BlurK bk;
};
void launch_resize_blur(const ResizeBlurArgs& a, hipStream_t s);
constexpr int kChainLevels = 8;
struct LevelChainArgs
{
    GrayBlurArgs g;
    ResizeBlurArgs lv[kChainLevels - 1];
    int n_lv;
    int G;
    int n_groups, groups_per_xcd;
    int frame0, n_frames;
};
bool launch_level_chain(const GrayBlurArgs& g, const ResizeBlurArgs* lv, int n_lv, int frames_per_group, int waves, int k6_max, hipStream_t s);
struct BlurWave
{
    int level;
    int item0;
    int generic;
    float inv_bsx;
};
void launch_blur(const uint8_t* d_pyr, uint8_t* d_blur, const Geometry& g, const BlurWave* d_waves, int wpf, int frame0, int n_frames,
                 hipStream_t s);
struct DescArgs
{
    const uint8_t* pyr;
    const uint8_t* blur;
    const uint32_t* sel;
    const uint32_t* sel_cnt;
    const uint32_t* orient_w;
    int cand_cap;
    int max_kp;
    float* xy;
    uint8_t* desc;
    int32_t* octave;
    float* angle;
    float* response;
    int32_t* count;
    uint32_t* flags;
    int n_frames = 0;
    const float* sel_resp = nullptr;
    uint8_t* h_mirror = nullptr;
    int cv_mode = 0;
};
void launch_describe(const Geometry& g, const DescArgs& a, int frame0, int n_frames, hipStream_t s);

struct ExactResizeArgs
{
    uint8_t* pyr;
    unsigned slab;
    int src_off, sw, sh, spitch, dst_off, dw, dh, dpitch;
    const int32_t* xofs;
    const uint32_t* xcoef;
    const int32_t* yofs;
    const uint32_t* ycoef;
    int xmin, xmax, ymin, ymax;
    int window12;
    int frame0;
};
void launch_resize_exact(const ExactResizeArgs& a, int n_frames, hipStream_t s);
struct CvSelectArgs
{
    uint32_t* cand;
    uint32_t* cand_cnt;
    uint32_t* tmp_kp;
    float* tmp_resp;
    uint32_t* sel;
    float* sel_resp;
    uint32_t* sel_cnt;
    uint32_t* flags;
    int cand_cap;
    int edge;
    int quota[kMaxLevels];
    int std_order;
};
constexpr int kSelLds = 4096;
constexpr int kSelLdsSmall = 1024;
void launch_zero_u32(uint32_t* p, int n, hipStream_t s);
void launch_fast_tiles(const uint8_t* d_pyr, const Geometry& g, int thr, const CvSelectArgs& a, int frame0, int n_frames,
                       hipStream_t s);
void launch_cv_select(const uint8_t* d_pyr, const Geometry& g, const CvSelectArgs& a, int frame0, int n_frames,
                      hipStream_t s);

struct MatchArgs
{
    const uint8_t* from_desc;
    const uint8_t* to_desc;
    long long from_stride, to_stride;
    const int32_t* from_cnt;
    const int32_t* to_cnt;
    int n_from_fixed, n_to_fixed;
    int cap;
    int32_t* idx0;
    int32_t* idx1;
    int32_t* dist0;
    int32_t* dist1;
    int cap_from = 0;
    int popcount_only = 0;
    uint32_t* partial = nullptr;
    int n_slices = 0;
    int n_pairs = 0, wg_per_pair = 0;
};
int launch_match_knn2(const MatchArgs& a, int n_pairs, hipStream_t s);
struct RatioArgs
{
    const int32_t* idx0;
    const int32_t* dist0;
    const int32_t* dist1;
    const int32_t* from_cnt;
    const int32_t* to_cnt;
    int n_from_fixed, n_to_fixed;
    int cap;
    const int32_t* thr;
    int32_t* from_idx;
    int32_t* to_idx;
    int32_t* n_out;
};
void launch_ratio_compact(const RatioArgs& a, int n_pairs, hipStream_t s);
bool launch_match_ratio_single(const MatchArgs& a, const RatioArgs& r, hipStream_t s);

}
```

modular-slam_amd/csrc/context.hpp:

```cpp
#pragma once
#include "common.hpp"
#include "devmem.hpp"
#include "../../include/mslam_hip.h"
#include <array>
#include <string>
#include <vector>

namespace mslam
{
struct BowState;
void bow_destroy(BowState*);
struct RelocState;
void reloc_destroy(RelocState*);
void set_blur_taps(const int* taps);
void build_blur_waves(const Geometry& g, int first_level, std::vector<BlurWave>& out);

struct StageTimer
{
    const char* name;
    hipEvent_t start, stop;
};
}

struct mslam_out_set
{
    mslam::DevBuf<float> xy;
    mslam::DevBuf<uint8_t> desc;
    mslam::DevBuf<int32_t> octave;
    mslam::DevBuf<float> angle, response;
    mslam::DevBuf<int32_t> count;
    mslam::DevBuf<int32_t> idx0, idx1, dist0, dist1;
    mslam::DevBuf<int32_t> mfrom, mto, mcount;
    hipEvent_t ev_detect = nullptr, ev_match = nullptr;
    bool match_pending = false;
};

struct mslam_hip_ctx
{
    mslam_hip_params p{};
    mslam::Geometry geom{};
    hipStream_t stream = nullptr;
    bool own_stream = false;
    int n_side = 2;
    hipStream_t side[4] = {nullptr, nullptr, nullptr, nullptr};
    hipEvent_t ev_fork = nullptr, ev_join[4] = {nullptr, nullptr, nullptr, nullptr};
    hipStream_t blur_stream[4] = {nullptr, nullptr, nullptr, nullptr};
    hipEvent_t ev_blur_fork[4] = {nullptr, nullptr, nullptr, nullptr}, ev_blur_join[4] = {nullptr, nullptr, nullptr, nullptr};
    bool fork_blur = false;
    std::string err;

    std::vector<mslam::CellDesc> cells;

    mslam::DevBuf<mslam::CellDesc> d_cells;
    mslam::DevBuf<int32_t> d_rs_ofs;
    mslam::DevBuf<uint32_t> d_rs_coef;
    std::vector<size_t> rs_x, rs_y;
    mslam::DevBuf<uint4> d_rs_qt;
    std::vector<size_t> rs_q;
    std::vector<int> rs_need;
    mslam::DevBuf<int32_t> d_cv_ofs;
    mslam::DevBuf<uint32_t> d_cv_coef;
    std::vector<size_t> cv_x, cv_y;
    std::vector<std::array<int, 4>> cv_range;
    std::vector<int> cv_window12;
    int cv_quota[mslam::kMaxLevels] = {0};
    mslam::DevBuf<int32_t> d_ratio_thr;
    mslam::DevBuf<uint32_t> d_orient_w;
    hipGraphExec_t detect_graph[2] = {nullptr, nullptr};
    bool use_graph = true;
    int cv_order = 0;
    bool mirror_results = false;
    hipGraphExec_t match_graph = nullptr;
    int match_graph_from_cap = 0, match_graph_to_cap = 0, match_graph_kind = -1, match_graph_kernel = 0;
    mslam::PinnedBuf<uint8_t> h_out;
    double ratio_cached = -1.0;

    mslam::DevBuf<uint8_t> d_stage;
    mslam::PinnedBuf<uint8_t> h_stage;
    mslam::DevBuf<uint8_t> d_pyr, d_blur;
    mslam::DevBuf<mslam::BlurWave> d_blur_waves;
    int blur_wpf = 0;
    int fused_levels = 0;
    int level_k6 = 9;
    bool knob_mirror_results = true, knob_zero_copy = true, knob_match_graph = true;
    size_t zero_copy_max_bytes = 1200000;
    int level_chain = 0, level_chain_frames = 2, level_chain_waves = 8, level_chain_k6 = 9;
    int level_k6_small = 1;
    mslam::DevBuf<uint32_t> d_cell_cnt, d_cell_kp;
    mslam::DevBuf<uint32_t> q_cand, q_cand_cnt, q_sel, q_sel_cnt, q_kp_node, q_ncnt_a, q_ncnt_b, q_child_cnt, q_ninfo, q_best;
    mslam::DevBuf<uint2> q_nodes_a, q_nodes_b;
    mslam::QuadArgs quad{};
    mslam::DevBuf<uint32_t> d_flags;

    mslam_out_set out[2];
    int cur = 0;
    hipStream_t stream_m = nullptr;
    bool overlap_match = true;
    int matcher_kind = 0;
    int last_match_kernel = 0;
    int n_last = 0;
    unsigned long long detect_seq = 0;
    unsigned long long points_seq = ~0ull;
    unsigned long long match_seq = ~0ull;
    bool have_prev = false;

    mslam::DevBuf<uint8_t> d_hm_from;
    uint8_t* d_hm_to = nullptr;
    mslam::DevBuf<int32_t> d_hm_out;
    int hm_from_cap = 0, hm_to_cap = 0;
    mslam::DevBuf<uint32_t> d_hm_partial;
    mslam::PinnedBuf<uint8_t> h_hm;

    mslam::DevBuf<double> d_xyz;
    mslam::DevBuf<uint8_t> d_valid;
    mslam::DevBuf<float> d_pnp_obj, d_pnp_img;
    mslam::DevBuf<int32_t> d_pnp_n, d_pnp_counts;
    mslam::DevBuf<double> d_pnp_hyp, d_pnp_out;
    mslam::DevBuf<uint8_t> d_pnp_mask;
    int pnp_iterations = 0;
    double pnp_confidence = 0.99;
    mslam::DevBuf<float> d_pnp1_obj, d_pnp1_img;
    mslam::DevBuf<double> d_pnp1_hyp, d_pnp1_out;
    mslam::DevBuf<int32_t> d_pnp1_counts;
    mslam::DevBuf<uint8_t> d_pnp1_mask;
    int pnp1_n_cap = 0, pnp1_it_cap = 0;
    mslam::DevBuf<double> d_mse1;
    bool pnp_attr_set = false;

    mslam::BowState* bow = nullptr;
    mslam::RelocState* reloc = nullptr;

    bool profiling = false;
    bool inplace_timing = false;
    std::vector<mslam::StageTimer> timers;
    size_t timers_used = 0;
};

#define MSLAM_CHK(c, call)                                                                                             \
    do                                                                                                                 \
    {                                                                                                                  \
        hipError_t e_ = (call);                                                                                        \
        if(e_ != hipSuccess)                                                                                           \
        {                                                                                                              \
            (c)->err = std::string(#call) + ": " + hipGetErrorString(e_);                                              \
            return MSLAM_HIP_E_RUNTIME;                                                                                \
        }                                                                                                              \
    } while(0)

namespace mslam
{
inline mslam_out_set& cur_out(mslam_hip_ctx* c) { return c->out[c->cur]; }

inline int fail(mslam_hip_ctx* c, int code, const std::string& msg)
{
    c->err = msg;
    return code;
}

struct StageScope
{
    mslam_hip_ctx* c;
    mslam::StageTimer* t = nullptr;
    hipStream_t st;
    StageScope(mslam_hip_ctx* ctx, const char* name, hipStream_t launch_stream = nullptr) : c(ctx)
    {
        if(!c->profiling && !c->inplace_timing)
            return;
        if(c->timers_used >= 8192)
            return;
        st = (c->profiling || !launch_stream) ? c->stream : launch_stream;
        if(c->timers_used == c->timers.size())
        {
            mslam::StageTimer nt{name, nullptr, nullptr};
            if(hipEventCreate(&nt.start) != hipSuccess || hipEventCreate(&nt.stop) != hipSuccess)
                return;
            c->timers.push_back(nt);
        }
        t = &c->timers[c->timers_used++];
        t->name = name;
        (void)hipEventRecord(t->start, st);
    }
    ~StageScope()
    {
        if(t)
            (void)hipEventRecord(t->stop, st);
    }
};

int bow_batch(mslam_hip_ctx* c, int add_to_db);

struct PnpBatchLaunch
{
    const float* obj;
    const float* img;
    const int32_t* n;
    int n_problems, cap;
    double fx, fy, cx, cy;
    int use_guess;
    double rvec[3], tvec[3];
    int iterations;
    double reprojection_error;
    unsigned long long seed;
    double* hyp;
    int32_t* counts;
    uint8_t* mask;
    double* out;
};
int pnp_launch_batch(mslam_hip_ctx* c, const PnpBatchLaunch& l);
void pnp_rotation_to_rvec(const double R[9], double rvec[3]);
}

extern "C" int mslam_ratio_table(mslam_hip_ctx* c, double ratio);
```

modular-slam_amd/csrc/k_level.hip:

```cpp
#include "common.hpp"
#include <cstdlib>
#include <type_traits>
#include <utility>

namespace mslam
{

typedef unsigned short u16x2_t __attribute__((ext_vector_type(2)));
typedef unsigned int u32x3 __attribute__((ext_vector_type(3)));
typedef decltype(__builtin_amdgcn_make_buffer_rsrc((void*)nullptr, (short)0, 0, 0)) BufRsrc;

__device__ __forceinline__ uint32_t lv_dot2u(uint32_t pair, uint32_t taps, uint32_t acc)
{
    u16x2_t a, b;
    a.x = (unsigned short)(pair & 0xFFFF);
    a.y = (unsigned short)(pair >> 16);
    b.x = (unsigned short)(taps & 0xFFFF);
    b.y = (unsigned short)(taps >> 16);
    return __builtin_amdgcn_udot2(a, b, acc, false);
}

constexpr uint32_t kDropLane = 0xFFFFFFF0u;

struct EdgeSel
{
    uint32_t selA, selB, selT, selU, maskT;
};
__device__ __forceinline__ EdgeSel edge_selectors(int x0, int w)
{
    EdgeSel e{0, 0, 0, 0, 0};
#pragma unroll
    for(int i = 0; i < 12; ++i)
    {
        int col = x0 - 4 + i;
        if(col < 0)
            col = -col;
        else if(col >= w)
            col = 2 * (w - 1) - col;
        int s = col - (x0 - 4);
        if(s < 0 || s > 11)
            s = i;
        const int b = i & 3;
        if(i < 4)
            e.selA |= (uint32_t)(s <= 7 ? s : i) << (8 * b);
        else if(i < 8)
            e.selB |= (uint32_t)(s <= 7 ? s : i) << (8 * b);
        else if(s < 4)
        {
            e.selT |= (uint32_t)s << (8 * b);
            e.maskT |= 0xFFu << (8 * b);
        }
        else
            e.selU |= (uint32_t)(s - 4) << (8 * b);
    }
    return e;
}

struct BlurRing
{
    uint32_t pr[6][4];
};

template <int PH, bool EMIT>
__device__ __forceinline__ uint32_t blur_feed(BlurRing& st, uint32_t B, const EdgeSel& e, const BlurK& k)
{
    const uint32_t L = (uint32_t)__builtin_amdgcn_update_dpp(0, (int)B, 0x138, 0xF, 0xF, true);
    const uint32_t R = (uint32_t)__builtin_amdgcn_update_dpp(0, (int)B, 0x130, 0xF, 0xF, true);
    const uint32_t A2 = __builtin_amdgcn_perm(B, L, e.selA);
    const uint32_t B2 = __builtin_amdgcn_perm(B, L, e.selB);
    const uint32_t T = __builtin_amdgcn_perm(B, L, e.selT);
    const uint32_t U = __builtin_amdgcn_perm(R, B, e.selU);
    uint32_t C2;
    asm("v_bfi_b32 %0, %1, %2, %3" : "=v"(C2) : "v"(e.maskT), "v"(T), "v"(U));
    uint32_t hv[4];
    hv[0] = __builtin_amdgcn_udot4(A2, k.ta[0], __builtin_amdgcn_udot4(B2, k.tb[0], 0u, false), false);
    hv[1] = __builtin_amdgcn_udot4(A2, k.ta[1], __builtin_amdgcn_udot4(B2, k.tb[1], __builtin_amdgcn_udot4(C2, k.tc[1], 0u, false), false), false);
    hv[2] = __builtin_amdgcn_udot4(A2, k.ta[2], __builtin_amdgcn_udot4(B2, k.tb[2], __builtin_amdgcn_udot4(C2, k.tc[2], 0u, false), false), false);
    hv[3] = __builtin_amdgcn_udot4(B2, k.tb[3], __builtin_amdgcn_udot4(C2, k.tc[3], 0u, false), false);
#pragma unroll
    for(int j = 0; j < 4; ++j)
        st.pr[(PH + 5) % 6][j] = __builtin_amdgcn_alignbit(hv[j], st.pr[(PH + 4) % 6][j], 16);
    uint32_t out = 0;
    if(EMIT)
    {
        uint32_t acc[4];
#pragma unroll
        for(int j = 0; j < 4; ++j)
        {
            acc[j] = lv_dot2u(st.pr[PH][j], k.t01, 32768u);
            acc[j] = lv_dot2u(st.pr[(PH + 2) % 6][j], k.t23, acc[j]);
            acc[j] = lv_dot2u(st.pr[(PH + 4) % 6][j], k.t45, acc[j]);
            acc[j] += __umul24(hv[j], k.t6);
        }
        out = __builtin_amdgcn_perm(acc[1], acc[0], 0x0C0C0602u) | __builtin_amdgcn_perm(acc[3], acc[2], 0x06020C0Cu);
    }
    return out;
}

__device__ __forceinline__ int reflect_row(int y, int h)
{
    const int ya = y < 0 ? -y : y;
    const int yb = 2 * (h - 1) - ya;
    return ya < yb ? ya : yb;
}

__device__ __forceinline__ uint32_t lv_gray_px(uint32_t c0, uint32_t c1, uint32_t c2)
{
    float v = __fadd_rn(__fmul_rn(0.299f, (float)c0), __fmul_rn(0.587f, (float)c1));
    v = __fadd_rn(v, __fmul_rn(0.114f, (float)c2));
    v = fminf(255.0f, v);
    return (uint32_t)(int)v;
}
__device__ __forceinline__ uint32_t lv_gray4(uint32_t a, uint32_t b, uint32_t c)
{
    const uint32_t p0 = lv_gray_px(a & 0xFF, (a >> 8) & 0xFF, (a >> 16) & 0xFF);
    const uint32_t p1 = lv_gray_px(a >> 24, b & 0xFF, (b >> 8) & 0xFF);
    const uint32_t p2 = lv_gray_px((b >> 16) & 0xFF, b >> 24, c & 0xFF);
    const uint32_t p3 = lv_gray_px((c >> 8) & 0xFF, (c >> 16) & 0xFF, c >> 24);
    return p0 | (p1 << 8) | (p2 << 16) | (p3 << 24);
}

struct Bgr3
{
    uint32_t a, b, c;
};

template <class F, int... I>
__device__ __forceinline__ void static_for(F&& f, std::integer_sequence<int, I...>)
{
    (f(std::integral_constant<int, I>{}), ...);
}

template <bool TILED, int DEEP>
__device__ __forceinline__ void gray_blur_wave(const GrayBlurArgs& a, const int gw, const int by)
{
    const int lane = threadIdx.x & 63;
    const int n_items = a.n_frames * a.quads;
    const int item_raw = gw * 62 - 1 + lane;
    if(gw * 62 >= n_items)
        return;
    const bool productive = lane >= 1 && lane <= 62 && item_raw < n_items;
    const int item = max(0, min(item_raw, n_items - 1));
    const int f = (int)(((float)item + 0.5f) * a.inv_quads);
    const int q = item - f * a.quads;
    const int R = 6 * a.k6 + 2;
    const int y0 = min(by * R, a.H - R);
    const EdgeSel e = edge_selectors(4 * q, a.W);
    const uint32_t src_v = (uint32_t)(f + a.frame0) * (uint32_t)(a.W * a.H * 3) + 12u * (uint32_t)q;
    const uint32_t col_v = (uint32_t)(f + a.frame0) * a.slab + 4u * (uint32_t)q;
    const uint32_t raw_v = productive ? col_v : kDropLane;
    const uint32_t blur_v = !productive ? kDropLane : TILED ? (uint32_t)(f + a.frame0) * a.slab + tiled_off((unsigned)a.pitch, 4 * q, 0) : col_v;
    const uint32_t n_rec = (uint32_t)(a.frame0 + a.n_frames) * a.slab;
    const BufRsrc blur_rs = __builtin_amdgcn_make_buffer_rsrc(a.blur, 0, (int)n_rec, 0x00020000);
    const uint32_t row_bytes = (uint32_t)a.W * 3u;

    const BufRsrc bgr_rs = __builtin_amdgcn_make_buffer_rsrc(const_cast<uint8_t*>(a.bgr), 0, -1, 0x00020000);
    auto load = [&](int i) {
        const int y = reflect_row(y0 - 3 + i, a.H);
        const u32x3 v = __builtin_amdgcn_raw_buffer_load_b96(bgr_rs, (int)src_v, (int)((uint32_t)y * row_bytes), 0);
        return Bgr3{v.x, v.y, v.z};
    };
    BlurRing st;
#pragma unroll
    for(int j = 0; j < 4; ++j)
        st.pr[4][j] = 0;
    auto compute = [&](auto ph, auto emit, auto sraw, int i, bool raw, const Bgr3& w) {
        constexpr int PH = decltype(ph)::value;
        constexpr bool EMIT = decltype(emit)::value;
        constexpr bool SRAW = decltype(sraw)::value;
        const uint32_t g = lv_gray4(w.a, w.b, w.c);
        if(SRAW)
            __builtin_amdgcn_raw_buffer_store_b32(g, __builtin_amdgcn_make_buffer_rsrc(a.pyr, 0, __builtin_amdgcn_readfirstlane(raw ? (int)n_rec : 0), 0x00020000),
                                                  (int)raw_v, (y0 - 3 + i) * a.pitch, 0);
        const uint32_t o = blur_feed<PH, EMIT>(st, g, e, a.bk);
        if(EMIT)
            __builtin_amdgcn_raw_buffer_store_b32(o, blur_rs, (int)blur_v,
                                                  (int)(TILED ? tiled_off((unsigned)a.pitch, 0, y0 - 6 + i) : (unsigned)((y0 - 6 + i) * a.pitch)), 0);
    };
    using std::integral_constant;
    if constexpr(DEEP > 0)
    {
        Bgr3 all[DEEP];
#pragma unroll
        for(int i = 0; i < DEEP; ++i)
            all[i] = load(i);
        __builtin_amdgcn_sched_barrier(0);
        static_for([&](auto ic) {
            constexpr int I = decltype(ic)::value;
            constexpr bool RAWROW = I >= 3 && I <= DEEP - 4;
            compute(integral_constant<int, I % 6>{}, integral_constant<bool, (I >= 6)>{}, integral_constant<bool, RAWROW>{}, I, RAWROW, all[I]);
        }, std::make_integer_sequence<int, DEEP>{});
        return;
    }
    Bgr3 ring[3];
    ring[0] = load(0);
    ring[1] = load(1);
    auto row = [&](auto ph, auto emit, auto sraw, int i, bool raw) {
        constexpr int PH = decltype(ph)::value;
        ring[(PH + 2) % 3] = load(min(i + 2, R + 5));
        compute(ph, emit, sraw, i, raw, ring[PH % 3]);
    };
#define MSLAM_ROW(PH, EMIT, SRAW, I, RAW) row(integral_constant<int, PH>{}, integral_constant<bool, EMIT>{}, integral_constant<bool, SRAW>{}, I, RAW)
    MSLAM_ROW(0, false, false, 0, false);
    MSLAM_ROW(1, false, false, 1, false);
    MSLAM_ROW(2, false, false, 2, false);
    MSLAM_ROW(3, false, true, 3, true);
    MSLAM_ROW(4, false, true, 4, true);
    MSLAM_ROW(5, false, true, 5, R > 2);
#pragma unroll 1
    for(int i0 = 6; i0 < R + 4; i0 += 6)
    {
        MSLAM_ROW(0, true, true, i0, true);
        MSLAM_ROW(1, true, true, i0 + 1, true);
        MSLAM_ROW(2, true, true, i0 + 2, true);
        MSLAM_ROW(3, true, true, i0 + 3, true);
        MSLAM_ROW(4, true, true, i0 + 4, true);
        MSLAM_ROW(5, true, true, i0 + 5, i0 + 5 < R + 3);
    }
    MSLAM_ROW(0, true, false, R + 4, false);
    MSLAM_ROW(1, true, false, R + 5, false);
#undef MSLAM_ROW
}

template <bool TILED, int DEEP>
__global__ __launch_bounds__(256) void k_gray_blur(GrayBlurArgs a)
{
    const int gw = __builtin_amdgcn_readfirstlane((int)((blockIdx.x & 7) * a.waves_per_xcd + (blockIdx.x >> 3) * 4 + (threadIdx.x >> 6)));
    gray_blur_wave<TILED, DEEP>(a, gw, (int)blockIdx.y);
}

struct Raw3
{
    uint32_t d0, d1, d2;
};
struct HRow
{
    uint32_t h[4];
};

template <bool EXACT, int NEED, bool TILED, int DEEP, bool COH>
__device__ __forceinline__ void resize_blur_wave(const ResizeBlurArgs& a, const int gw, const int by)
{
    const int lane = threadIdx.x & 63;
    const int n_items = a.n_frames * a.quads;
    const int R = 6 * a.k6 + 2;
    const int y0 = min(by * R, a.dh - R);
    const int my_row = reflect_row(y0 - 3 + min(lane, R + 5), a.dh);
    const int my_y0 = a.yofs[my_row];
    const uint32_t my_yc = a.ycoef[my_row];
    if(gw * 62 >= n_items)
        return;
    const int item_raw = gw * 62 - 1 + lane;
    const bool productive = lane >= 1 && lane <= 62 && item_raw < n_items;
    const int item = max(0, min(item_raw, n_items - 1));
    const int f = (int)(((float)item + 0.5f) * a.inv_quads);
    const int qx = item - f * a.quads;
    const EdgeSel e = edge_selectors(4 * qx, a.dw);
    const uint4 t0 = a.qt[3 * qx], t1 = a.qt[3 * qx + 1], t2 = a.qt[3 * qx + 2];
    const uint32_t sel[4] = {t0.z, t0.w, t1.x, t1.y}, coef[4] = {t1.z, t1.w, t2.x, t2.y};
    const uint32_t src_v = (uint32_t)(f + a.frame0) * a.slab + t0.x;
    const uint32_t col_v = (uint32_t)(f + a.frame0) * a.slab + (uint32_t)a.dst_off + 4u * (uint32_t)qx;
    const uint32_t raw_v = productive ? col_v : kDropLane;
    const uint32_t blur_v = !productive ? kDropLane
                            : TILED   ? (uint32_t)(f + a.frame0) * a.slab + (uint32_t)a.dst_off + tiled_off((unsigned)a.dpitch, 4 * qx, 0)
                                      : col_v;
    const uint32_t n_rec = (uint32_t)(a.frame0 + a.n_frames) * a.slab;
    const BufRsrc blur_rs = __builtin_amdgcn_make_buffer_rsrc(a.blur, 0, (int)n_rec, 0x00020000);
    const uint8_t* src_lv = a.pyr + a.src_off;

    const BufRsrc src_rs = __builtin_amdgcn_make_buffer_rsrc(const_cast<uint8_t*>(src_lv), 0, -1, 0x00020000);
    auto load = [&](int sy) {
        const u32x3 v = __builtin_amdgcn_raw_buffer_load_b96(src_rs, (int)src_v, (int)((uint32_t)sy * (uint32_t)a.spitch), COH ? 1 : 0);
        return Raw3{v.x, v.y, v.z};
    };
    auto load_if = [&](int sy, bool need) {
        const BufRsrc rs = __builtin_amdgcn_make_buffer_rsrc(const_cast<uint8_t*>(src_lv), 0, __builtin_amdgcn_readfirstlane(need ? -1 : 0), 0x00020000);
        const u32x3 v = __builtin_amdgcn_raw_buffer_load_b96(rs, (int)src_v, (int)((uint32_t)sy * (uint32_t)a.spitch), COH ? 1 : 0);
        return Raw3{v.x, v.y, v.z};
    };
    auto hinterp = [&](const Raw3& w) {
        HRow r;
#pragma unroll
        for(int k = 0; k < 4; ++k)
        {
            uint32_t lo = w.d0, hi = w.d1;
            if(NEED & (1 << k))
            {
                const bool up = (t0.y >> k) & 1u;
                lo = up ? w.d1 : w.d0;
                hi = up ? w.d2 : w.d1;
            }
            const uint32_t pr = __builtin_amdgcn_perm(hi, lo, sel[k]);
            u16x2_t pv, cv;
            pv.x = (unsigned short)(pr & 0xFFFF);
            pv.y = (unsigned short)(pr >> 16);
            cv.x = (unsigned short)(coef[k] & 0xFFFF);
            cv.y = (unsigned short)(coef[k] >> 16);
            r.h[k] = EXACT ? __builtin_amdgcn_udot2(pv, cv, 0u, false) : __builtin_amdgcn_udot2(pv, cv, 0u, false) >> 4;
        }
        return r;
    };
    auto rows_of = [&](int i, int& sy0, int& sy1) {
        const int t = __builtin_amdgcn_readlane(my_y0, i);
        sy0 = max(0, min(t, a.sh - 1));
        sy1 = max(0, min(t + 1, a.sh - 1));
    };

    BlurRing st;
#pragma unroll
    for(int j = 0; j < 4; ++j)
        st.pr[4][j] = 0;
    HRow hA{}, hB{};
    int rowA = -1, rowB = -1;
    auto compute = [&](auto ph, auto emit, auto sraw, int i, bool raw, int sy0, int sy1, const Raw3& wA, const Raw3& wB) {
        constexpr int PH = decltype(ph)::value;
        constexpr bool EMIT = decltype(emit)::value;
        constexpr bool SRAW = decltype(sraw)::value;
        const bool reuse = sy1 == rowB && (sy0 == rowA || sy0 == rowB);
        if(!reuse)
        {
            if(sy0 == rowB)
            {
                asm volatile("");
                hA = hB;
            }
            else
            {
                asm volatile("");
                hA = hinterp(wA);
            }
            rowA = sy0;
            if(sy1 == sy0)
            {
                asm volatile("");
                hB = hA;
            }
            else
            {
                asm volatile("");
                hB = hinterp(wB);
            }
            rowB = sy1;
        }
        const uint32_t yc = (uint32_t)__builtin_amdgcn_readlane((int)my_yc, i);
        const uint32_t b0 = yc & 0xFFFF, b1 = yc >> 16;
        auto blend = [&](const HRow& h0, const HRow& h1) {
            uint32_t r = 0;
            if(EXACT)
            {
                uint32_t acc[4];
#pragma unroll
                for(int k = 0; k < 4; ++k)
                    acc[k] = __umul24(b1, h1.h[k]) + (__umul24(b0, h0.h[k]) + 32768u);
                r = __builtin_amdgcn_perm(acc[1], acc[0], 0x0C0C0602u) | __builtin_amdgcn_perm(acc[3], acc[2], 0x06020C0Cu);
            }
            else
            {
                const uint32_t b0s = b0 << 16, b1s = b1 << 16;
                uint32_t v[4];
#pragma unroll
                for(int k = 0; k < 4; ++k)
                    v[k] = __umulhi(h0.h[k], b0s) + __umulhi(h1.h[k], b1s) + 2u;
                const uint32_t p01 = (v[0] | (v[1] << 16)) >> 2, p23 = (v[2] | (v[3] << 16)) >> 2;
                r = __builtin_amdgcn_perm(p23, p01, 0x06040200u);
            }
            return r;
        };
        uint32_t g;
        if(sy0 == rowA)
        {
            asm volatile("");
            g = blend(hA, hB);
        }
        else
        {
            asm volatile("");
            g = blend(hB, hB);
        }
        if(SRAW)
            __builtin_amdgcn_raw_buffer_store_b32(g, __builtin_amdgcn_make_buffer_rsrc(a.pyr, 0, __builtin_amdgcn_readfirstlane(raw ? (int)n_rec : 0), 0x00020000),
                                                  (int)raw_v, (y0 - 3 + i) * a.dpitch, 0);
        const uint32_t o = blur_feed<PH, EMIT>(st, g, e, a.bk);
        if(EMIT)
            __builtin_amdgcn_raw_buffer_store_b32(o, blur_rs, (int)blur_v,
                                                  (int)(TILED ? tiled_off((unsigned)a.dpitch, 0, y0 - 6 + i) : (unsigned)((y0 - 6 + i) * a.dpitch)), 0);
    };
    using std::integral_constant;
    if constexpr(DEEP > 0)
    {
        Raw3 allA[DEEP], allB[DEEP];
#pragma unroll
        for(int i = 0; i < DEEP; ++i)
        {
            int y0i, y1i;
            rows_of(i, y0i, y1i);
            allA[i] = load(y0i);
            allB[i] = load(y1i);
        }
        __builtin_amdgcn_sched_barrier(0);
        static_for([&](auto ic) {
            constexpr int I = decltype(ic)::value;
            constexpr bool RAWROW = I >= 3 && I <= DEEP - 4;
            int sy0, sy1;
            rows_of(I, sy0, sy1);
            compute(integral_constant<int, I % 6>{}, integral_constant<bool, (I >= 6)>{}, integral_constant<bool, RAWROW>{}, I, RAWROW, sy0, sy1,
                    allA[I], allB[I]);
        }, std::make_integer_sequence<int, DEEP>{});
        return;
    }
    Raw3 RA[3], RB[3];
    int c0_y0, c0_y1, c1_y0, c1_y1;
    rows_of(0, c0_y0, c0_y1);
    rows_of(1, c1_y0, c1_y1);
    RA[0] = load(c0_y0);
    RB[0] = load(c0_y1);
    RA[1] = load(c1_y0);
    RB[1] = load(c1_y1);
    auto row = [&](auto ph, auto emit, auto sraw, int i, bool raw) {
        constexpr int PH = decltype(ph)::value;
        const int sy0 = c0_y0, sy1 = c0_y1;
        {
            int ny0, ny1;
            rows_of(min(i + 2, R + 5), ny0, ny1);
            RA[(PH + 2) % 3] = load_if(ny0, ny0 != c1_y1 || a.always_load);
            RB[(PH + 2) % 3] = load(ny1);
            c0_y0 = c1_y0, c0_y1 = c1_y1;
            c1_y0 = ny0, c1_y1 = ny1;
        }
        compute(ph, emit, sraw, i, raw, sy0, sy1, RA[PH % 3], RB[PH % 3]);
    };
#define MSLAM_ROW(PH, EMIT, SRAW, I, RAW) row(integral_constant<int, PH>{}, integral_constant<bool, EMIT>{}, integral_constant<bool, SRAW>{}, I, RAW)
    MSLAM_ROW(0, false, false, 0, false);
    MSLAM_ROW(1, false, false, 1, false);
    MSLAM_ROW(2, false, false, 2, false);
    MSLAM_ROW(3, false, true, 3, true);
    MSLAM_ROW(4, false, true, 4, true);
    MSLAM_ROW(5, false, true, 5, R > 2);
#pragma unroll 1
    for(int i0 = 6; i0 < R + 4; i0 += 6)
    {
        MSLAM_ROW(0, true, true, i0, true);
        MSLAM_ROW(1, true, true, i0 + 1, true);
        MSLAM_ROW(2, true, true, i0 + 2, true);
        MSLAM_ROW(3, true, true, i0 + 3, true);
        MSLAM_ROW(4, true, true, i0 + 4, true);
        MSLAM_ROW(5, true, true, i0 + 5, i0 + 5 < R + 3);
    }
    MSLAM_ROW(0, true, false, R + 4, false);
    MSLAM_ROW(1, true, false, R + 5, false);
#undef MSLAM_ROW
}

template <bool EXACT, int NEED, bool TILED, int DEEP>
__global__ __launch_bounds__(256) void k_resize_blur(ResizeBlurArgs a)
{
    const int gw = __builtin_amdgcn_readfirstlane((int)((blockIdx.x & 7) * a.waves_per_xcd + (blockIdx.x >> 3) * 4 + (threadIdx.x >> 6)));
    resize_blur_wave<EXACT, NEED, TILED, DEEP, false>(a, gw, (int)blockIdx.y);
}

template <bool EXACT, int NEED, bool TILED, int WAVES, bool COH>
__global__ __launch_bounds__(WAVES * 64) void k_level_chain(LevelChainArgs ch)
{
    const int grp = (int)(blockIdx.x & 7) * ch.groups_per_xcd + (int)(blockIdx.x >> 3);
    if(grp >= ch.n_groups)
        return;
    const int wave = __builtin_amdgcn_readfirstlane((int)(threadIdx.x >> 6));
    const int f0 = grp * ch.G;
    const int nf = min(ch.G, ch.n_frames - f0);
    {
        GrayBlurArgs a = ch.g;
        a.frame0 = ch.frame0 + f0;
        a.n_frames = nf;
        const int R = 6 * a.k6 + 2;
        const int nwx = (nf * a.quads + 61) / 62, nby = (a.H + R - 1) / R;
#pragma unroll 1
        for(int item = wave; item < nwx * nby; item += WAVES)
        {
            const int by = item / nwx;
            gray_blur_wave<TILED, 0>(a, item - by * nwx, by);
        }
    }
#pragma unroll 1
    for(int l = 0; l < ch.n_lv; ++l)
    {
        __builtin_amdgcn_fence(__ATOMIC_RELEASE, "workgroup");
        __syncthreads();
        __builtin_amdgcn_fence(__ATOMIC_ACQUIRE, "workgroup");
        ResizeBlurArgs a = ch.lv[l];
        a.frame0 = ch.frame0 + f0;
        a.n_frames = nf;
        const int R = 6 * a.k6 + 2;
        const int nwx = (nf * a.quads + 61) / 62, nby = (a.dh + R - 1) / R;
#pragma unroll 1
        for(int item = wave; item < nwx * nby; item += WAVES)
        {
            const int by = item / nwx;
            resize_blur_wave<EXACT, NEED, TILED, 0, COH>(a, item - by * nwx, by);
        }
    }
}

static int chain_k6(int quads, int rows, int G, int waves, int k6_max)
{
    const long nwx = ((long)G * quads + 61) / 62;
    int best = 1;
    long best_cost = -1;
    for(int k = 1; k <= k6_max && 6 * k + 2 <= rows; ++k)
    {
        const int R = 6 * k + 2;
        const long items = nwx * ((rows + R - 1) / R);
        const long cost = ((items + waves - 1) / waves) * (R + 6);
        if(best_cost < 0 || cost <= best_cost)
            best = k, best_cost = cost;
    }
    return best;
}

bool launch_level_chain(const GrayBlurArgs& g, const ResizeBlurArgs* lv, int n_lv, int frames_per_group, int waves, int k6_max, hipStream_t s)
{
    if(n_lv > kChainLevels - 1 || !g.blur_tiled)
        return false;
    LevelChainArgs ch{};
    ch.g = g;
    ch.G = frames_per_group;
    ch.frame0 = g.frame0;
    ch.n_frames = g.n_frames;
    ch.n_lv = n_lv;
    ch.g.k6 = chain_k6(g.quads, g.H, ch.G, waves, k6_max);
    int need = 0;
    for(int l = 0; l < n_lv; ++l)
    {
        if(lv[l].exact || !lv[l].blur_tiled)
            return false;
        ch.lv[l] = lv[l];
        ch.lv[l].always_load = 0;
        ch.lv[l].k6 = chain_k6(lv[l].quads, lv[l].dh, ch.G, waves, k6_max);
        need |= lv[l].need_mask;
    }
    ch.n_groups = (g.n_frames + ch.G - 1) / ch.G;
    ch.groups_per_xcd = (ch.n_groups + 7) / 8;
    const dim3 grid(8 * ch.groups_per_xcd);
    const bool n8 = (need & ~8) == 0;
#define MSLAM_LC(N, W) hipLaunchKernelGGL((k_level_chain<false, N, true, W, true>), grid, dim3(W * 64), 0, s, ch)
    if(waves == 8)
    {
        if(n8) MSLAM_LC(8, 8); else MSLAM_LC(15, 8);
    }
    else
    {
        if(n8) MSLAM_LC(8, 4); else MSLAM_LC(15, 4);
    }
#undef MSLAM_LC
    return true;
}

void launch_resize_blur(const ResizeBlurArgs& a, hipStream_t s)
{
    const int R = 6 * a.k6 + 2;
    const int n_waves = (a.n_frames * a.quads + 61) / 62;
    ResizeBlurArgs b = a;
    b.waves_per_xcd = ((n_waves + 31) / 32) * 4;
    dim3 grid(8 * (b.waves_per_xcd / 4), (a.dh + R - 1) / R);
    const int need = (a.need_mask & ~8) == 0 ? (a.need_mask ? 8 : 0) : (a.need_mask & ~12) == 0 ? 12 : 15;
    static const bool deep_env = [] { const char* e = getenv("MSLAM_HIP_LEVEL_DEEP"); return !e || atoi(e) != 0; }();
    const int deep = (a.always_load && deep_env && a.k6 <= 1) ? R + 6 : 0;
#define MSLAM_RB3(E, N, T) do { if(deep == 8) hipLaunchKernelGGL((k_resize_blur<E, N, T, 8>), grid, dim3(256), 0, s, b); \
                               else if(deep == 14) hipLaunchKernelGGL((k_resize_blur<E, N, T, 14>), grid, dim3(256), 0, s, b); \
                               else hipLaunchKernelGGL((k_resize_blur<E, N, T, 0>), grid, dim3(256), 0, s, b); } while(0)
#define MSLAM_RB(E, N) do { if(a.blur_tiled) MSLAM_RB3(E, N, true); else MSLAM_RB3(E, N, false); } while(0)
    if(a.exact)
    {
        if(need == 0) MSLAM_RB(true, 0); else if(need == 8) MSLAM_RB(true, 8); else if(need == 12) MSLAM_RB(true, 12); else MSLAM_RB(true, 15);
    }
    else
    {
        if(need == 0) MSLAM_RB(false, 0); else if(need == 8) MSLAM_RB(false, 8); else if(need == 12) MSLAM_RB(false, 12); else MSLAM_RB(false, 15);
    }
#undef MSLAM_RB3
#undef MSLAM_RB
}

void launch_gray_blur(const GrayBlurArgs& a, hipStream_t s)
{
    const int R = 6 * a.k6 + 2;
    const int n_waves = (a.n_frames * a.quads + 61) / 62;
    GrayBlurArgs b = a;
    b.waves_per_xcd = ((n_waves + 31) / 32) * 4;
    dim3 grid(8 * (b.waves_per_xcd / 4), (a.H + R - 1) / R);
    static const bool deep_env = [] { const char* e = getenv("MSLAM_HIP_LEVEL_DEEP"); return !e || atoi(e) != 0; }();
    const int deep = (a.n_frames < 8 && deep_env && a.k6 <= 1) ? R + 6 : 0;
#define MSLAM_GB(T) do { if(deep == 8) hipLaunchKernelGGL((k_gray_blur<T, 8>), grid, dim3(256), 0, s, b); \
                        else if(deep == 14) hipLaunchKernelGGL((k_gray_blur<T, 14>), grid, dim3(256), 0, s, b); \
                        else hipLaunchKernelGGL((k_gray_blur<T, 0>), grid, dim3(256), 0, s, b); } while(0)
    if(a.blur_tiled)
        MSLAM_GB(true);
    else
        MSLAM_GB(false);
#undef MSLAM_GB
}

}
```

Baseline: 625.9 million.

## Process eight pixels per lane in gray/resize-blur kernels for large batches

Adds an eight-pixel-per-lane variant of the gray-conversion and resize+blur kernels, with a new host-built octet resize table. For batches of at least 8 frames it halves the lane count per row, loads wider source windows and uses 64-bit stores, and shares neighbour pixels between the two quads without DPP exchanges. This amortises per-lane index and table work but raises register pressure and restricts which resize patterns qualify. The default level_k6 row-block depth also drops from 9 to 5.

```diff
diff --git a/modular-slam_amd/csrc/api.hip b/modular-slam_amd/csrc/api.hip
--- a/modular-slam_amd/csrc/api.hip
+++ b/modular-slam_amd/csrc/api.hip
@@ -413,6 +413,48 @@
     need_out = need;
 }
 
+static void build_oct_table(const std::vector<int32_t>& ofs, const std::vector<uint32_t>& coef, size_t x0, int dw,
+                            std::vector<uint4>& qt, size_t& start_out)
+{
+    static const int dword_of[8] = {0, 0, 0, 0, 1, 1, 1, 2};
+    const int no = (dw + 7) / 8;
+    const size_t start = qt.size() / 5;
+    bool ok = true;
+    for(int o = 0; o < no && ok; ++o)
+    {
+        const uint32_t base = (uint32_t)ofs[x0 + 8 * o] & ~3u;
+        uint32_t sel[8], cf[8], flags = 0;
+        for(int k = 0; k < 8; ++k)
+        {
+            const int dx = std::min(8 * o + k, dw - 1);
+            const int shift = ofs[x0 + dx] - (int)base;
+            const uint32_t a0 = coef[x0 + dx] & 0xFFFF, a1 = coef[x0 + dx] >> 16;
+            if(a0 > 0xFFF || a1 > 0xFFF)
+                ok = false;
+            int m = dword_of[k];
+            bool fits = shift >= 4 * m && shift <= 4 * m + 6;
+            if(!fits && ((kOctNeed >> k) & 1) && shift >= 4 * m + 4 && shift <= 4 * m + 10)
+                ++m, flags |= 1u << k, fits = true;
+            if(!fits && 8 * o + k < dw)
+                ok = false;
+            sel[k] = 0x0c010c00u + (uint32_t)(fits ? shift - 4 * m : 0) * 0x00010001u;
+            cf[k] = a0 | (a1 << 16);
+        }
+        qt.push_back(make_uint4(base, flags, sel[0], sel[1]));
+        qt.push_back(make_uint4(sel[2], sel[3], sel[4], sel[5]));
+        qt.push_back(make_uint4(sel[6], sel[7], cf[0], cf[1]));
+        qt.push_back(make_uint4(cf[2], cf[3], cf[4], cf[5]));
+        qt.push_back(make_uint4(cf[6], cf[7], 0, 0));
+    }
+    if(!ok)
+    {
+        qt.resize(start * 5);
+        start_out = SIZE_MAX;
+        return;
+    }
+    start_out = start;
+}
+
 static int create_impl(mslam_hip_ctx* c)
 {
     const mslam_hip_params& p = c->p;
@@ -511,6 +553,13 @@
             qt.push_back(make_uint4(0, 0, 0, 0));
             MSLAM_CHK(c, c->d_rs_qt.alloc(qt.size()));
             MSLAM_CHK(c, hipMemcpy(c->d_rs_qt, qt.data(), qt.size() * 16, hipMemcpyHostToDevice));
+            std::vector<uint4> qt8;
+            c->rs_q8.assign(p.n_levels, SIZE_MAX);
+            for(int l = 1; l < p.n_levels; ++l)
+                build_oct_table(ofs, coef, c->cv_x[l], g.lv[l].w, qt8, c->rs_q8[l]);
+            qt8.push_back(make_uint4(0, 0, 0, 0));
+            MSLAM_CHK(c, c->d_rs_qt8.alloc(qt8.size()));
+            MSLAM_CHK(c, hipMemcpy(c->d_rs_qt8, qt8.data(), qt8.size() * 16, hipMemcpyHostToDevice));
         }
         ofs.push_back(0);
         coef.push_back(0);
@@ -543,6 +592,13 @@
         qt.push_back(make_uint4(0, 0, 0, 0));
         MSLAM_CHK(c, c->d_rs_qt.alloc(qt.size()));
         MSLAM_CHK(c, hipMemcpy(c->d_rs_qt, qt.data(), qt.size() * 16, hipMemcpyHostToDevice));
+        std::vector<uint4> qt8;
+        c->rs_q8.assign(p.n_levels, SIZE_MAX);
+        for(int l = 1; l < p.n_levels; ++l)
+            build_oct_table(ofs, coef, c->rs_x[l], g.lv[l].w, qt8, c->rs_q8[l]);
+        qt8.push_back(make_uint4(0, 0, 0, 0));
+        MSLAM_CHK(c, c->d_rs_qt8.alloc(qt8.size()));
+        MSLAM_CHK(c, hipMemcpy(c->d_rs_qt8, qt8.data(), qt8.size() * 16, hipMemcpyHostToDevice));
         ofs.push_back(0);
         coef.push_back(0);
         MSLAM_CHK(c, c->d_rs_ofs.alloc(ofs.size()));
@@ -599,7 +655,7 @@
                     c->level_chain_waves = 8;
                 c->level_chain_k6 = lk ? std::max(1, std::min(9, atoi(lk))) : 9;
             }
-            c->level_k6 = k ? std::max(1, atoi(k)) : 9;
+            c->level_k6 = k ? std::max(1, atoi(k)) : 5;
             const bool fits = (p.width & 3) == 0 && (double)B * p.width * p.height * 3 < 4294967296.0 &&
                               (double)B * g.slab < 4294901760.0  && (size_t)B * (p.width / 4) < (1u << 22) && p.height >= 8;
             int n_fused = fits ? 1 : 0;
@@ -788,11 +844,12 @@
     ra.slab = g.slab;
     ra.src_off = sl.offset, ra.sh = sl.h, ra.spitch = sl.pitch;
     ra.dst_off = dl.offset, ra.dw = dl.w, ra.dh = dl.h, ra.dpitch = dl.pitch;
-    ra.qt = c->d_rs_qt + 3 * c->rs_q[l];
+    ra.wide = nf >= 8 && !chain_out && c->rs_q8[l] != SIZE_MAX ? 1 : 0;
+    ra.qt = ra.wide ? c->d_rs_qt8 + 5 * c->rs_q8[l] : c->d_rs_qt + 3 * c->rs_q[l];
     ra.yofs = yofs;
     ra.ycoef = ycoef;
     ra.frame0 = f0, ra.n_frames = nf;
-    ra.quads = (dl.w + 3) / 4;
+    ra.quads = ra.wide ? (dl.w + 7) / 8 : (dl.w + 3) / 4;
     ra.inv_quads = 1.0f / (float)ra.quads;
     if(k6 == 0 && dl.h >= 380)
         k6 = 1;
@@ -865,7 +922,8 @@
                 ga.W = g.W, ga.H = g.H, ga.pitch = g.lv[0].pitch;
                 ga.slab = g.slab;
                 ga.n_frames = nf, ga.frame0 = f0;
-                ga.quads = g.W / 4;
+                ga.wide = nf >= 8 ? 1 : 0;
+                ga.quads = ga.wide ? (g.W + 7) / 8 : g.W / 4;
                 ga.inv_quads = 1.0f / (float)ga.quads;
                 ga.k6 = std::max(k6_batch == 0 && g.H < 380 ? 0 : 1, std::min(k6_batch, (g.H - 2) / 6));
                 ga.blur_tiled = g.blur_tiled;
diff --git a/modular-slam_amd/csrc/common.hpp b/modular-slam_amd/csrc/common.hpp
--- a/modular-slam_amd/csrc/common.hpp
+++ b/modular-slam_amd/csrc/common.hpp
@@ -143,6 +143,7 @@
     int n_frames, frame0;
     int quads;
     float inv_quads;
+    int wide;
     int k6;
     int waves_per_xcd;
     int blur_tiled;
@@ -161,6 +162,7 @@
     int frame0, n_frames;
     int quads;
     float inv_quads;
+    int wide;
     int k6;
     int need_mask;
     int exact;
@@ -170,6 +172,7 @@
     BlurK bk;
 };
 void launch_resize_blur(const ResizeBlurArgs& a, hipStream_t s);
+constexpr int kOctNeed = 0x48;
 constexpr int kChainLevels = 8;
 struct LevelChainArgs
 {
diff --git a/modular-slam_amd/csrc/context.hpp b/modular-slam_amd/csrc/context.hpp
--- a/modular-slam_amd/csrc/context.hpp
+++ b/modular-slam_amd/csrc/context.hpp
@@ -58,6 +58,8 @@
     mslam::DevBuf<uint4> d_rs_qt;
     std::vector<size_t> rs_q;
     std::vector<int> rs_need;
+    mslam::DevBuf<uint4> d_rs_qt8;
+    std::vector<size_t> rs_q8;
     mslam::DevBuf<int32_t> d_cv_ofs;
     mslam::DevBuf<uint32_t> d_cv_coef;
     std::vector<size_t> cv_x, cv_y;
@@ -81,7 +83,7 @@
     mslam::DevBuf<mslam::BlurWave> d_blur_waves;
     int blur_wpf = 0;
     int fused_levels = 0;
-    int level_k6 = 9;
+    int level_k6 = 5;
     bool knob_mirror_results = true, knob_zero_copy = true, knob_match_graph = true;
     size_t zero_copy_max_bytes = 1200000;
     int level_chain = 0, level_chain_frames = 2, level_chain_waves = 8, level_chain_k6 = 9;
diff --git a/modular-slam_amd/csrc/k_level.hip b/modular-slam_amd/csrc/k_level.hip
--- a/modular-slam_amd/csrc/k_level.hip
+++ b/modular-slam_amd/csrc/k_level.hip
@@ -7,7 +7,9 @@
 {
 
 typedef unsigned short u16x2_t __attribute__((ext_vector_type(2)));
+typedef unsigned int u32x2 __attribute__((ext_vector_type(2)));
 typedef unsigned int u32x3 __attribute__((ext_vector_type(3)));
+typedef unsigned int u32x4 __attribute__((ext_vector_type(4)));
 typedef decltype(__builtin_amdgcn_make_buffer_rsrc((void*)nullptr, (short)0, 0, 0)) BufRsrc;
 
 __device__ __forceinline__ uint32_t lv_dot2u(uint32_t pair, uint32_t taps, uint32_t acc)
@@ -56,45 +58,70 @@
     return e;
 }
 
+template <int NQ>
 struct BlurRing
 {
-    uint32_t pr[6][4];
+    uint32_t pr[6][4 * NQ];
 };
 
-template <int PH, bool EMIT>
-__device__ __forceinline__ uint32_t blur_feed(BlurRing& st, uint32_t B, const EdgeSel& e, const BlurK& k)
-{
-    const uint32_t L = (uint32_t)__builtin_amdgcn_update_dpp(0, (int)B, 0x138, 0xF, 0xF, true);
-    const uint32_t R = (uint32_t)__builtin_amdgcn_update_dpp(0, (int)B, 0x130, 0xF, 0xF, true);
+__device__ __forceinline__ void hblur4(uint32_t L, uint32_t B, uint32_t R, const EdgeSel& e, const BlurK& k, uint32_t* hv)
+{
     const uint32_t A2 = __builtin_amdgcn_perm(B, L, e.selA);
     const uint32_t B2 = __builtin_amdgcn_perm(B, L, e.selB);
     const uint32_t T = __builtin_amdgcn_perm(B, L, e.selT);
     const uint32_t U = __builtin_amdgcn_perm(R, B, e.selU);
     uint32_t C2;
     asm("v_bfi_b32 %0, %1, %2, %3" : "=v"(C2) : "v"(e.maskT), "v"(T), "v"(U));
-    uint32_t hv[4];
     hv[0] = __builtin_amdgcn_udot4(A2, k.ta[0], __builtin_amdgcn_udot4(B2, k.tb[0], 0u, false), false);
     hv[1] = __builtin_amdgcn_udot4(A2, k.ta[1], __builtin_amdgcn_udot4(B2, k.tb[1], __builtin_amdgcn_udot4(C2, k.tc[1], 0u, false), false), false);
     hv[2] = __builtin_amdgcn_udot4(A2, k.ta[2], __builtin_amdgcn_udot4(B2, k.tb[2], __builtin_amdgcn_udot4(C2, k.tc[2], 0u, false), false), false);
     hv[3] = __builtin_amdgcn_udot4(B2, k.tb[3], __builtin_amdgcn_udot4(C2, k.tc[3], 0u, false), false);
-#pragma unroll
-    for(int j = 0; j < 4; ++j)
+}
+
+template <int PH, bool EMIT, int NQ>
+__device__ __forceinline__ void blur_feed(BlurRing<NQ>& st, const uint32_t (&B)[NQ], const EdgeSel (&e)[NQ], const BlurK& k, uint32_t (&out)[NQ])
+{
+    const uint32_t L = (uint32_t)__builtin_amdgcn_update_dpp(0, (int)B[NQ - 1], 0x138, 0xF, 0xF, true);
+    const uint32_t R = (uint32_t)__builtin_amdgcn_update_dpp(0, (int)B[0], 0x130, 0xF, 0xF, true);
+    uint32_t hv[4 * NQ];
+#pragma unroll
+    for(int q = 0; q < NQ; ++q)
+        hblur4(q == 0 ? L : B[q > 0 ? q - 1 : 0], B[q], q == NQ - 1 ? R : B[q < NQ - 1 ? q + 1 : q], e[q], k, hv + 4 * q);
+#pragma unroll
+    for(int j = 0; j < 4 * NQ; ++j)
         st.pr[(PH + 5) % 6][j] = __builtin_amdgcn_alignbit(hv[j], st.pr[(PH + 4) % 6][j], 16);
-    uint32_t out = 0;
+#pragma unroll
+    for(int q = 0; q < NQ; ++q)
+        out[q] = 0;
     if(EMIT)
     {
-        uint32_t acc[4];
-#pragma unroll
-        for(int j = 0; j < 4; ++j)
+        uint32_t acc[4 * NQ];
+#pragma unroll
+        for(int j = 0; j < 4 * NQ; ++j)
         {
             acc[j] = lv_dot2u(st.pr[PH][j], k.t01, 32768u);
             acc[j] = lv_dot2u(st.pr[(PH + 2) % 6][j], k.t23, acc[j]);
             acc[j] = lv_dot2u(st.pr[(PH + 4) % 6][j], k.t45, acc[j]);
             acc[j] += __umul24(hv[j], k.t6);
         }
-        out = __builtin_amdgcn_perm(acc[1], acc[0], 0x0C0C0602u) | __builtin_amdgcn_perm(acc[3], acc[2], 0x06020C0Cu);
-    }
-    return out;
+#pragma unroll
+        for(int q = 0; q < NQ; ++q)
+            out[q] = __builtin_amdgcn_perm(acc[4 * q + 1], acc[4 * q], 0x0C0C0602u) | __builtin_amdgcn_perm(acc[4 * q + 3], acc[4 * q + 2], 0x06020C0Cu);
+    }
+}
+
+template <int NQ>
+__device__ __forceinline__ void store_quads(const uint32_t (&v)[NQ], BufRsrc rs, uint32_t voff, uint32_t soff)
+{
+    static_assert(NQ == 1 || NQ == 2, "lane width");
+    if constexpr(NQ == 1)
+        __builtin_amdgcn_raw_buffer_store_b32(v[0], rs, (int)voff, (int)soff, 0);
+    else
+    {
+        u32x2 p;
+        p.x = v[0], p.y = v[1];
+        __builtin_amdgcn_raw_buffer_store_b64(p, rs, (int)voff, (int)soff, 0);
+    }
 }
 
 __device__ __forceinline__ int reflect_row(int y, int h)
@@ -131,9 +158,10 @@
     (f(std::integral_constant<int, I>{}), ...);
 }
 
-template <bool TILED, int DEEP>
+template <bool TILED, int DEEP, int NQ>
 __device__ __forceinline__ void gray_blur_wave(const GrayBlurArgs& a, const int gw, const int by)
 {
+    static_assert(DEEP == 0 || NQ == 1, "the deep-prefetch instances are 4-pixel walks");
     const int lane = threadIdx.x & 63;
     const int n_items = a.n_frames * a.quads;
     const int item_raw = gw * 62 - 1 + lane;
@@ -143,44 +171,63 @@
     const int item = max(0, min(item_raw, n_items - 1));
     const int f = (int)(((float)item + 0.5f) * a.inv_quads);
     const int q = item - f * a.quads;
+    const int x0 = 4 * NQ * q;
     const int R = 6 * a.k6 + 2;
     const int y0 = min(by * R, a.H - R);
-    const EdgeSel e = edge_selectors(4 * q, a.W);
-    const uint32_t src_v = (uint32_t)(f + a.frame0) * (uint32_t)(a.W * a.H * 3) + 12u * (uint32_t)q;
-    const uint32_t col_v = (uint32_t)(f + a.frame0) * a.slab + 4u * (uint32_t)q;
+    EdgeSel e[NQ];
+    uint32_t src_v[NQ];
+#pragma unroll
+    for(int j = 0; j < NQ; ++j)
+    {
+        e[j] = edge_selectors(x0 + 4 * j, a.W);
+        src_v[j] = (uint32_t)(f + a.frame0) * (uint32_t)(a.W * a.H * 3) + 3u * (uint32_t)(x0 + 4 * j < a.W ? x0 + 4 * j : x0);
+    }
+    const uint32_t col_v = (uint32_t)(f + a.frame0) * a.slab + (uint32_t)x0;
     const uint32_t raw_v = productive ? col_v : kDropLane;
-    const uint32_t blur_v = !productive ? kDropLane : TILED ? (uint32_t)(f + a.frame0) * a.slab + tiled_off((unsigned)a.pitch, 4 * q, 0) : col_v;
+    const uint32_t blur_v = !productive ? kDropLane : TILED ? (uint32_t)(f + a.frame0) * a.slab + tiled_off((unsigned)a.pitch, x0, 0) : col_v;
     const uint32_t n_rec = (uint32_t)(a.frame0 + a.n_frames) * a.slab;
     const BufRsrc blur_rs = __builtin_amdgcn_make_buffer_rsrc(a.blur, 0, (int)n_rec, 0x00020000);
     const uint32_t row_bytes = (uint32_t)a.W * 3u;
 
     const BufRsrc bgr_rs = __builtin_amdgcn_make_buffer_rsrc(const_cast<uint8_t*>(a.bgr), 0, -1, 0x00020000);
+    struct BgrRow
+    {
+        Bgr3 q[NQ];
+    };
     auto load = [&](int i) {
         const int y = reflect_row(y0 - 3 + i, a.H);
-        const u32x3 v = __builtin_amdgcn_raw_buffer_load_b96(bgr_rs, (int)src_v, (int)((uint32_t)y * row_bytes), 0);
-        return Bgr3{v.x, v.y, v.z};
-    };
-    BlurRing st;
-#pragma unroll
-    for(int j = 0; j < 4; ++j)
+        BgrRow r;
+#pragma unroll
+        for(int j = 0; j < NQ; ++j)
+        {
+            const u32x3 v = __builtin_amdgcn_raw_buffer_load_b96(bgr_rs, (int)src_v[j], (int)((uint32_t)y * row_bytes), 0);
+            r.q[j] = Bgr3{v.x, v.y, v.z};
+        }
+        return r;
+    };
+    BlurRing<NQ> st;
+#pragma unroll
+    for(int j = 0; j < 4 * NQ; ++j)
         st.pr[4][j] = 0;
-    auto compute = [&](auto ph, auto emit, auto sraw, int i, bool raw, const Bgr3& w) {
+    auto compute = [&](auto ph, auto emit, auto sraw, int i, bool raw, const BgrRow& w) {
         constexpr int PH = decltype(ph)::value;
         constexpr bool EMIT = decltype(emit)::value;
         constexpr bool SRAW = decltype(sraw)::value;
-        const uint32_t g = lv_gray4(w.a, w.b, w.c);
+        uint32_t g[NQ], o[NQ];
+#pragma unroll
+        for(int j = 0; j < NQ; ++j)
+            g[j] = lv_gray4(w.q[j].a, w.q[j].b, w.q[j].c);
         if(SRAW)
-            __builtin_amdgcn_raw_buffer_store_b32(g, __builtin_amdgcn_make_buffer_rsrc(a.pyr, 0, __builtin_amdgcn_readfirstlane(raw ? (int)n_rec : 0), 0x00020000),
-                                                  (int)raw_v, (y0 - 3 + i) * a.pitch, 0);
-        const uint32_t o = blur_feed<PH, EMIT>(st, g, e, a.bk);
+            store_quads<NQ>(g, __builtin_amdgcn_make_buffer_rsrc(a.pyr, 0, __builtin_amdgcn_readfirstlane(raw ? (int)n_rec : 0), 0x00020000), raw_v,
+                            (uint32_t)((y0 - 3 + i) * a.pitch));
+        blur_feed<PH, EMIT, NQ>(st, g, e, a.bk, o);
         if(EMIT)
-            __builtin_amdgcn_raw_buffer_store_b32(o, blur_rs, (int)blur_v,
-                                                  (int)(TILED ? tiled_off((unsigned)a.pitch, 0, y0 - 6 + i) : (unsigned)((y0 - 6 + i) * a.pitch)), 0);
+            store_quads<NQ>(o, blur_rs, blur_v, TILED ? tiled_off((unsigned)a.pitch, 0, y0 - 6 + i) : (unsigned)((y0 - 6 + i) * a.pitch));
     };
     using std::integral_constant;
     if constexpr(DEEP > 0)
     {
-        Bgr3 all[DEEP];
+        BgrRow all[DEEP];
 #pragma unroll
         for(int i = 0; i < DEEP; ++i)
             all[i] = load(i);
@@ -192,7 +239,7 @@
         }, std::make_integer_sequence<int, DEEP>{});
         return;
     }
-    Bgr3 ring[3];
+    BgrRow ring[3];
     ring[0] = load(0);
     ring[1] = load(1);
     auto row = [&](auto ph, auto emit, auto sraw, int i, bool raw) {
@@ -222,25 +269,31 @@
 #undef MSLAM_ROW
 }
 
-template <bool TILED, int DEEP>
+template <bool TILED, int DEEP, int NQ>
 __global__ __launch_bounds__(256) void k_gray_blur(GrayBlurArgs a)
 {
     const int gw = __builtin_amdgcn_readfirstlane((int)((blockIdx.x & 7) * a.waves_per_xcd + (blockIdx.x >> 3) * 4 + (threadIdx.x >> 6)));
-    gray_blur_wave<TILED, DEEP>(a, gw, (int)blockIdx.y);
-}
-
-struct Raw3
-{
-    uint32_t d0, d1, d2;
+    gray_blur_wave<TILED, DEEP, NQ>(a, gw, (int)blockIdx.y);
+}
+
+template <int NQ>
+struct SrcWin
+{
+    uint32_t d[NQ + 2];
 };
+template <int NQ>
 struct HRow
 {
-    uint32_t h[4];
+    uint32_t h[4 * NQ];
 };
-
-template <bool EXACT, int NEED, bool TILED, int DEEP, bool COH>
+__device__ __forceinline__ constexpr int oct_dword(int k) { return k < 4 ? 0 : k < 7 ? 1 : 2; }
+
+template <bool EXACT, int NEED, bool TILED, int DEEP, bool COH, int NQ>
 __device__ __forceinline__ void resize_blur_wave(const ResizeBlurArgs& a, const int gw, const int by)
 {
+    static_assert(DEEP == 0 || NQ == 1, "the deep-prefetch instances are 4-pixel walks");
+    static_assert(NQ == 1 || (NEED & ~kOctNeed) == 0, "an eight-pixel window has two stepping pixels");
+    constexpr int NP = 4 * NQ;
     const int lane = threadIdx.x & 63;
     const int n_items = a.n_frames * a.quads;
     const int R = 6 * a.k6 + 2;
@@ -255,40 +308,67 @@
     const int item = max(0, min(item_raw, n_items - 1));
     const int f = (int)(((float)item + 0.5f) * a.inv_quads);
     const int qx = item - f * a.quads;
-    const EdgeSel e = edge_selectors(4 * qx, a.dw);
-    const uint4 t0 = a.qt[3 * qx], t1 = a.qt[3 * qx + 1], t2 = a.qt[3 * qx + 2];
-    const uint32_t sel[4] = {t0.z, t0.w, t1.x, t1.y}, coef[4] = {t1.z, t1.w, t2.x, t2.y};
-    const uint32_t src_v = (uint32_t)(f + a.frame0) * a.slab + t0.x;
-    const uint32_t col_v = (uint32_t)(f + a.frame0) * a.slab + (uint32_t)a.dst_off + 4u * (uint32_t)qx;
+    const int x0 = NP * qx;
+    EdgeSel e[NQ];
+#pragma unroll
+    for(int j = 0; j < NQ; ++j)
+        e[j] = edge_selectors(x0 + 4 * j, a.dw);
+    uint32_t sel[NP], coef[NP], win_off, up_flags;
+    if constexpr(NQ == 1)
+    {
+        const uint4 t0 = a.qt[3 * qx], t1 = a.qt[3 * qx + 1], t2 = a.qt[3 * qx + 2];
+        win_off = t0.x, up_flags = t0.y;
+        sel[0] = t0.z, sel[1] = t0.w, sel[2] = t1.x, sel[3] = t1.y;
+        coef[0] = t1.z, coef[1] = t1.w, coef[2] = t2.x, coef[3] = t2.y;
+    }
+    else
+    {
+        const uint4 t0 = a.qt[5 * qx], t1 = a.qt[5 * qx + 1], t2 = a.qt[5 * qx + 2], t3 = a.qt[5 * qx + 3], t4 = a.qt[5 * qx + 4];
+        win_off = t0.x, up_flags = t0.y;
+        sel[0] = t0.z, sel[1] = t0.w, sel[2] = t1.x, sel[3] = t1.y, sel[4] = t1.z, sel[5] = t1.w, sel[6] = t2.x, sel[7] = t2.y;
+        coef[0] = t2.z, coef[1] = t2.w, coef[2] = t3.x, coef[3] = t3.y, coef[4] = t3.z, coef[5] = t3.w, coef[6] = t4.x, coef[7] = t4.y;
+    }
+    const uint32_t src_v = (uint32_t)(f + a.frame0) * a.slab + win_off;
+    const uint32_t col_v = (uint32_t)(f + a.frame0) * a.slab + (uint32_t)a.dst_off + (uint32_t)x0;
     const uint32_t raw_v = productive ? col_v : kDropLane;
     const uint32_t blur_v = !productive ? kDropLane
-                            : TILED   ? (uint32_t)(f + a.frame0) * a.slab + (uint32_t)a.dst_off + tiled_off((unsigned)a.dpitch, 4 * qx, 0)
+                            : TILED   ? (uint32_t)(f + a.frame0) * a.slab + (uint32_t)a.dst_off + tiled_off((unsigned)a.dpitch, x0, 0)
                                       : col_v;
     const uint32_t n_rec = (uint32_t)(a.frame0 + a.n_frames) * a.slab;
     const BufRsrc blur_rs = __builtin_amdgcn_make_buffer_rsrc(a.blur, 0, (int)n_rec, 0x00020000);
     const uint8_t* src_lv = a.pyr + a.src_off;
 
+    auto load_rs = [&](BufRsrc rs, int sy) {
+        SrcWin<NQ> w;
+        if constexpr(NQ == 1)
+        {
+            const u32x3 v = __builtin_amdgcn_raw_buffer_load_b96(rs, (int)src_v, (int)((uint32_t)sy * (uint32_t)a.spitch), COH ? 1 : 0);
+            w.d[0] = v.x, w.d[1] = v.y, w.d[2] = v.z;
+        }
+        else
+        {
+            const u32x4 v = __builtin_amdgcn_raw_buffer_load_b128(rs, (int)src_v, (int)((uint32_t)sy * (uint32_t)a.spitch), COH ? 1 : 0);
+            w.d[0] = v.x, w.d[1] = v.y, w.d[2] = v.z, w.d[3] = v.w;
+        }
+        return w;
+    };
     const BufRsrc src_rs = __builtin_amdgcn_make_buffer_rsrc(const_cast<uint8_t*>(src_lv), 0, -1, 0x00020000);
-    auto load = [&](int sy) {
-        const u32x3 v = __builtin_amdgcn_raw_buffer_load_b96(src_rs, (int)src_v, (int)((uint32_t)sy * (uint32_t)a.spitch), COH ? 1 : 0);
-        return Raw3{v.x, v.y, v.z};
-    };
+    auto load = [&](int sy) { return load_rs(src_rs, sy); };
     auto load_if = [&](int sy, bool need) {
-        const BufRsrc rs = __builtin_amdgcn_make_buffer_rsrc(const_cast<uint8_t*>(src_lv), 0, __builtin_amdgcn_readfirstlane(need ? -1 : 0), 0x00020000);
-        const u32x3 v = __builtin_amdgcn_raw_buffer_load_b96(rs, (int)src_v, (int)((uint32_t)sy * (uint32_t)a.spitch), COH ? 1 : 0);
-        return Raw3{v.x, v.y, v.z};
-    };
-    auto hinterp = [&](const Raw3& w) {
-        HRow r;
-#pragma unroll
-        for(int k = 0; k < 4; ++k)
-        {
-            uint32_t lo = w.d0, hi = w.d1;
+        return load_rs(__builtin_amdgcn_make_buffer_rsrc(const_cast<uint8_t*>(src_lv), 0, __builtin_amdgcn_readfirstlane(need ? -1 : 0), 0x00020000), sy);
+    };
+    auto hinterp = [&](const SrcWin<NQ>& w) {
+        HRow<NQ> r;
+#pragma unroll
+        for(int k = 0; k < NP; ++k)
+        {
+            const int m = NQ == 1 ? 0 : oct_dword(k);
+            uint32_t lo = w.d[m], hi = w.d[m + 1];
             if(NEED & (1 << k))
             {
-                const bool up = (t0.y >> k) & 1u;
-                lo = up ? w.d1 : w.d0;
-                hi = up ? w.d2 : w.d1;
+                const bool up = (up_flags >> k) & 1u;
+                lo = up ? w.d[m + 1] : w.d[m];
+                hi = up ? w.d[m + 2 < NQ + 2 ? m + 2 : m + 1] : w.d[m + 1];
             }
             const uint32_t pr = __builtin_amdgcn_perm(hi, lo, sel[k]);
             u16x2_t pv, cv;
@@ -306,13 +386,13 @@
         sy1 = max(0, min(t + 1, a.sh - 1));
     };
 
-    BlurRing st;
-#pragma unroll
-    for(int j = 0; j < 4; ++j)
+    BlurRing<NQ> st;
+#pragma unroll
+    for(int j = 0; j < NP; ++j)
         st.pr[4][j] = 0;
-    HRow hA{}, hB{};
+    HRow<NQ> hA{}, hB{};
     int rowA = -1, rowB = -1;
-    auto compute = [&](auto ph, auto emit, auto sraw, int i, bool raw, int sy0, int sy1, const Raw3& wA, const Raw3& wB) {
+    auto compute = [&](auto ph, auto emit, auto sraw, int i, bool raw, int sy0, int sy1, const SrcWin<NQ>& wA, const SrcWin<NQ>& wB) {
         constexpr int PH = decltype(ph)::value;
         constexpr bool EMIT = decltype(emit)::value;
         constexpr bool SRAW = decltype(sraw)::value;
@@ -344,51 +424,52 @@
         }
         const uint32_t yc = (uint32_t)__builtin_amdgcn_readlane((int)my_yc, i);
         const uint32_t b0 = yc & 0xFFFF, b1 = yc >> 16;
-        auto blend = [&](const HRow& h0, const HRow& h1) {
-            uint32_t r = 0;
-            if(EXACT)
+        auto blend = [&](const HRow<NQ>& h0, const HRow<NQ>& h1, uint32_t (&r)[NQ]) {
+#pragma unroll
+            for(int j = 0; j < NQ; ++j)
             {
-                uint32_t acc[4];
-#pragma unroll
-                for(int k = 0; k < 4; ++k)
-                    acc[k] = __umul24(b1, h1.h[k]) + (__umul24(b0, h0.h[k]) + 32768u);
-                r = __builtin_amdgcn_perm(acc[1], acc[0], 0x0C0C0602u) | __builtin_amdgcn_perm(acc[3], acc[2], 0x06020C0Cu);
+                if(EXACT)
+                {
+                    uint32_t acc[4];
+#pragma unroll
+                    for(int k = 0; k < 4; ++k)
+                        acc[k] = __umul24(b1, h1.h[4 * j + k]) + (__umul24(b0, h0.h[4 * j + k]) + 32768u);
+                    r[j] = __builtin_amdgcn_perm(acc[1], acc[0], 0x0C0C0602u) | __builtin_amdgcn_perm(acc[3], acc[2], 0x06020C0Cu);
+                }
+                else
+                {
+                    const uint32_t b0s = b0 << 16, b1s = b1 << 16;
+                    uint32_t v[4];
+#pragma unroll
+                    for(int k = 0; k < 4; ++k)
+                        v[k] = __umulhi(h0.h[4 * j + k], b0s) + __umulhi(h1.h[4 * j + k], b1s) + 2u;
+                    const uint32_t p01 = (v[0] | (v[1] << 16)) >> 2, p23 = (v[2] | (v[3] << 16)) >> 2;
+                    r[j] = __builtin_amdgcn_perm(p23, p01, 0x06040200u);
+                }
             }
-            else
-            {
-                const uint32_t b0s = b0 << 16, b1s = b1 << 16;
-                uint32_t v[4];
-#pragma unroll
-                for(int k = 0; k < 4; ++k)
-                    v[k] = __umulhi(h0.h[k], b0s) + __umulhi(h1.h[k], b1s) + 2u;
-                const uint32_t p01 = (v[0] | (v[1] << 16)) >> 2, p23 = (v[2] | (v[3] << 16)) >> 2;
-                r = __builtin_amdgcn_perm(p23, p01, 0x06040200u);
-            }
-            return r;
         };
-        uint32_t g;
+        uint32_t g[NQ], o[NQ];
         if(sy0 == rowA)
         {
             asm volatile("");
-            g = blend(hA, hB);
+            blend(hA, hB, g);
         }
         else
         {
             asm volatile("");
-            g = blend(hB, hB);
+            blend(hB, hB, g);
         }
         if(SRAW)
-            __builtin_amdgcn_raw_buffer_store_b32(g, __builtin_amdgcn_make_buffer_rsrc(a.pyr, 0, __builtin_amdgcn_readfirstlane(raw ? (int)n_rec : 0), 0x00020000),
-                                                  (int)raw_v, (y0 - 3 + i) * a.dpitch, 0);
-        const uint32_t o = blur_feed<PH, EMIT>(st, g, e, a.bk);
+            store_quads<NQ>(g, __builtin_amdgcn_make_buffer_rsrc(a.pyr, 0, __builtin_amdgcn_readfirstlane(raw ? (int)n_rec : 0), 0x00020000), raw_v,
+                            (uint32_t)((y0 - 3 + i) * a.dpitch));
+        blur_feed<PH, EMIT, NQ>(st, g, e, a.bk, o);
         if(EMIT)
-            __builtin_amdgcn_raw_buffer_store_b32(o, blur_rs, (int)blur_v,
-                                                  (int)(TILED ? tiled_off((unsigned)a.dpitch, 0, y0 - 6 + i) : (unsigned)((y0 - 6 + i) * a.dpitch)), 0);
+            store_quads<NQ>(o, blur_rs, blur_v, TILED ? tiled_off((unsigned)a.dpitch, 0, y0 - 6 + i) : (unsigned)((y0 - 6 + i) * a.dpitch));
     };
     using std::integral_constant;
     if constexpr(DEEP > 0)
     {
-        Raw3 allA[DEEP], allB[DEEP];
+        SrcWin<NQ> allA[DEEP], allB[DEEP];
 #pragma unroll
         for(int i = 0; i < DEEP; ++i)
         {
@@ -408,7 +489,7 @@
         }, std::make_integer_sequence<int, DEEP>{});
         return;
     }
-    Raw3 RA[3], RB[3];
+    SrcWin<NQ> RA[3], RB[3];
     int c0_y0, c0_y1, c1_y0, c1_y1;
     rows_of(0, c0_y0, c0_y1);
     rows_of(1, c1_y0, c1_y1);
@@ -451,11 +532,11 @@
 #undef MSLAM_ROW
 }
 
-template <bool EXACT, int NEED, bool TILED, int DEEP>
+template <bool EXACT, int NEED, bool TILED, int DEEP, int NQ>
 __global__ __launch_bounds__(256) void k_resize_blur(ResizeBlurArgs a)
 {
     const int gw = __builtin_amdgcn_readfirstlane((int)((blockIdx.x & 7) * a.waves_per_xcd + (blockIdx.x >> 3) * 4 + (threadIdx.x >> 6)));
-    resize_blur_wave<EXACT, NEED, TILED, DEEP, false>(a, gw, (int)blockIdx.y);
+    resize_blur_wave<EXACT, NEED, TILED, DEEP, false, NQ>(a, gw, (int)blockIdx.y);
 }
 
 template <bool EXACT, int NEED, bool TILED, int WAVES, bool COH>
@@ -477,7 +558,7 @@
         for(int item = wave; item < nwx * nby; item += WAVES)
         {
             const int by = item / nwx;
-            gray_blur_wave<TILED, 0>(a, item - by * nwx, by);
+            gray_blur_wave<TILED, 0, 1>(a, item - by * nwx, by);
         }
     }
 #pragma unroll 1
@@ -495,7 +576,7 @@
         for(int item = wave; item < nwx * nby; item += WAVES)
         {
             const int by = item / nwx;
-            resize_blur_wave<EXACT, NEED, TILED, 0, COH>(a, item - by * nwx, by);
+            resize_blur_wave<EXACT, NEED, TILED, 0, COH, 1>(a, item - by * nwx, by);
         }
     }
 }
@@ -561,12 +642,20 @@
     ResizeBlurArgs b = a;
     b.waves_per_xcd = ((n_waves + 31) / 32) * 4;
     dim3 grid(8 * (b.waves_per_xcd / 4), (a.dh + R - 1) / R);
+    if(a.wide)
+    {
+#define MSLAM_RB8(E) do { if(a.blur_tiled) hipLaunchKernelGGL((k_resize_blur<E, kOctNeed, true, 0, 2>), grid, dim3(256), 0, s, b); \
+                         else hipLaunchKernelGGL((k_resize_blur<E, kOctNeed, false, 0, 2>), grid, dim3(256), 0, s, b); } while(0)
+        if(a.exact) MSLAM_RB8(true); else MSLAM_RB8(false);
+#undef MSLAM_RB8
+        return;
+    }
     const int need = (a.need_mask & ~8) == 0 ? (a.need_mask ? 8 : 0) : (a.need_mask & ~12) == 0 ? 12 : 15;
     static const bool deep_env = [] { const char* e = getenv("MSLAM_HIP_LEVEL_DEEP"); return !e || atoi(e) != 0; }();
     const int deep = (a.always_load && deep_env && a.k6 <= 1) ? R + 6 : 0;
-#define MSLAM_RB3(E, N, T) do { if(deep == 8) hipLaunchKernelGGL((k_resize_blur<E, N, T, 8>), grid, dim3(256), 0, s, b); \
-                               else if(deep == 14) hipLaunchKernelGGL((k_resize_blur<E, N, T, 14>), grid, dim3(256), 0, s, b); \
-                               else hipLaunchKernelGGL((k_resize_blur<E, N, T, 0>), grid, dim3(256), 0, s, b); } while(0)
+#define MSLAM_RB3(E, N, T) do { if(deep == 8) hipLaunchKernelGGL((k_resize_blur<E, N, T, 8, 1>), grid, dim3(256), 0, s, b); \
+                               else if(deep == 14) hipLaunchKernelGGL((k_resize_blur<E, N, T, 14, 1>), grid, dim3(256), 0, s, b); \
+                               else hipLaunchKernelGGL((k_resize_blur<E, N, T, 0, 1>), grid, dim3(256), 0, s, b); } while(0)
 #define MSLAM_RB(E, N) do { if(a.blur_tiled) MSLAM_RB3(E, N, true); else MSLAM_RB3(E, N, false); } while(0)
     if(a.exact)
     {
@@ -587,11 +676,19 @@
     GrayBlurArgs b = a;
     b.waves_per_xcd = ((n_waves + 31) / 32) * 4;
     dim3 grid(8 * (b.waves_per_xcd / 4), (a.H + R - 1) / R);
+    if(a.wide)
+    {
+        if(a.blur_tiled)
+            hipLaunchKernelGGL((k_gray_blur<true, 0, 2>), grid, dim3(256), 0, s, b);
+        else
+            hipLaunchKernelGGL((k_gray_blur<false, 0, 2>), grid, dim3(256), 0, s, b);
+        return;
+    }
     static const bool deep_env = [] { const char* e = getenv("MSLAM_HIP_LEVEL_DEEP"); return !e || atoi(e) != 0; }();
     const int deep = (a.n_frames < 8 && deep_env && a.k6 <= 1) ? R + 6 : 0;
-#define MSLAM_GB(T) do { if(deep == 8) hipLaunchKernelGGL((k_gray_blur<T, 8>), grid, dim3(256), 0, s, b); \
-                        else if(deep == 14) hipLaunchKernelGGL((k_gray_blur<T, 14>), grid, dim3(256), 0, s, b); \
-                        else hipLaunchKernelGGL((k_gray_blur<T, 0>), grid, dim3(256), 0, s, b); } while(0)
+#define MSLAM_GB(T) do { if(deep == 8) hipLaunchKernelGGL((k_gray_blur<T, 8, 1>), grid, dim3(256), 0, s, b); \
+                        else if(deep == 14) hipLaunchKernelGGL((k_gray_blur<T, 14, 1>), grid, dim3(256), 0, s, b); \
+                        else hipLaunchKernelGGL((k_gray_blur<T, 0, 1>), grid, dim3(256), 0, s, b); } while(0)
     if(a.blur_tiled)
         MSLAM_GB(true);
     else
```

Result: faster. 638.8 million, median of 6 (+2.1%).
